# yunjinli/TRASE

Measured on AMD Instinct MI355X. Metric: views/sec (fwd+bwd), 1080p, 300k Gaussians, 32-d feat, higher is better.
Workload: dtype f32 (channel contractions: 3-product bf16-split MFMA, fp32 accumulate)

## Files before the change

include/trase_rast.h:

```cpp
#ifndef TRASE_RAST_H
#define TRASE_RAST_H

#include <stddef.h>
#include <stdint.h>

#ifdef __cplusplus
extern "C" {
#endif

typedef void* trase_stream_t;

enum {
  TRASE_OK = 0,
  TRASE_ERR_INVALID = -1,
  TRASE_ERR_UNSUPPORTED = -2,
  TRASE_ERR_WORKSPACE = -3,
  TRASE_ERR_HIP = -4
};

typedef struct TraseRastSettings {
  int32_t image_height;
  int32_t image_width;
  float tanfovx;
  float tanfovy;
  const float* bg;
  float scale_modifier;
  const float* viewmatrix;
  const float* projmatrix;
  int32_t sh_degree;
  const float* campos;
  int32_t prefiltered;
  int32_t debug;
  int32_t device;
  int32_t variant;
  int32_t tile_row_begin;
  int32_t tile_row_end;
  float feat_bg;
  int32_t reserved0;
} TraseRastSettings;

typedef enum TraseVariant {
  TRASE_VARIANT_DEPTH_GRAD = 0x100,
  TRASE_VARIANT_FEATS_BG = 0x10000,
  TRASE_VARIANT_DEPTH_NORM = 0x20000,
  TRASE_VARIANT_FEATURES_ONLY_BWD = 0x400,
  TRASE_VARIANT_VALU_BACKWARD = 0x40,
  TRASE_VARIANT_VALU_FORWARD = 0x2000,
  TRASE_VARIANT_SLOT_LISTS = 0x100000,
  TRASE_VARIANT_DEPTH32 = 0x400000,
  TRASE_VARIANT_FORWARD_ONLY = 0x800000,
  TRASE_VARIANT_SPARSE_STRIP_GRADS = 0x200000,
  TRASE_VARIANT_AB_TIMING = 0x1000,
  TRASE_VARIANT_AB_COUNT = 0x8000,
  TRASE_VARIANT_AB_ORDER_IMAGE = 0x40000,
  TRASE_VARIANT_AB_ORDER_8 = 0x80000
} TraseVariant;

typedef struct TraseRastInputs {
  int32_t P;
  int32_t M;
  int32_t F;
  const float* means3D;
  const float* shs;
  const float* sh_objs;
  const float* colors_precomp;
  const float* opacities;
  const float* scales;
  const float* rotations;
  const float* cov3D_precomp;
} TraseRastInputs;

typedef struct TraseRastOutputs {
  float* image;
  int32_t* radii;
  float* feats;
  float* depth;
} TraseRastOutputs;

typedef struct TraseRastWorkspace {
  void* geom; size_t geom_bytes;
  void* bin;  size_t bin_bytes;
  void* img;  size_t img_bytes;
  void* pre;  size_t pre_bytes;
  void* tmp;  size_t tmp_bytes;
  int64_t capacity;
} TraseRastWorkspace;

typedef struct TraseRastSizes {
  size_t geom_bytes, bin_bytes, img_bytes, pre_bytes, tmp_bytes, bwd_tmp_bytes;
} TraseRastSizes;

typedef struct TraseRastGrads {
  const float* dL_dimage;
  const float* dL_dfeats;
  const float* dL_ddepth;
  float* dL_dmeans3D;
  float* dL_dmeans2D;
  float* dL_dshs;
  float* dL_dsh_objs;
  float* dL_dcolors;
  float* dL_dopacities;
  float* dL_dscales;
  float* dL_drotations;
  float* dL_dcov3D;
} TraseRastGrads;

int trase_rast_sizes(int32_t P, int32_t W, int32_t H, int32_t F, int64_t capacity, TraseRastSizes* out);

int trase_rast_preprocess(const TraseRastSettings* s, const TraseRastInputs* in, const TraseRastOutputs* out,
                          const TraseRastWorkspace* ws, trase_stream_t stream);

int trase_rast_status(const TraseRastWorkspace* ws, int64_t status[3], trase_stream_t stream);

int trase_rast_geom_layout(int32_t P, int64_t off[6]);

int trase_rast_render(const TraseRastSettings* s, const TraseRastInputs* in, const TraseRastOutputs* out,
                      const TraseRastWorkspace* ws, trase_stream_t stream);

int trase_rast_forward(const TraseRastSettings* s, const TraseRastInputs* in, const TraseRastOutputs* out,
                       const TraseRastWorkspace* ws, trase_stream_t stream);

int trase_rast_backward(const TraseRastSettings* s, const TraseRastInputs* in, const TraseRastOutputs* out,
                        const TraseRastWorkspace* ws, const TraseRastGrads* g, trase_stream_t stream);

typedef struct TraseRastRawInputs {
  int32_t P;
  int32_t F;
  int32_t norm_features;
  const float* xyz;
  const float* d_xyz;
  const float* features_dc;
  const float* features_rest;
  const float* opacity;
  const float* scaling;
  const float* d_scaling;
  const float* rotation;
  const float* d_rotation;
  const float* gaussian_features;
  float* featn;
  const float* colors_precomp;
  const uint8_t* mask;
  const float* d_xyz_se3;
  int32_t sh_dir_undeformed;
  int32_t reserved1;
} TraseRastRawInputs;

typedef struct TraseRastRawGrads {
  const float* dL_dimage; const float* dL_dfeats; const float* dL_ddepth;
  float* dL_dxyz; float* dL_dd_xyz; float* dL_dmeans2D;
  float* dL_dfeatures_dc; float* dL_dfeatures_rest; float* dL_dopacity;
  float* dL_dscaling; float* dL_dd_scaling; float* dL_drotation; float* dL_dd_rotation;
  float* dL_dgaussian_features;
  float* dL_dcolors_precomp;
  float* dL_dd_xyz_se3;
} TraseRastRawGrads;

int trase_rast_preprocess_raw(const TraseRastSettings* s, const TraseRastRawInputs* raw, const TraseRastOutputs* out,
                              const TraseRastWorkspace* ws, trase_stream_t stream);
int trase_rast_render_raw(const TraseRastSettings* s, const TraseRastRawInputs* raw, const TraseRastOutputs* out,
                          const TraseRastWorkspace* ws, trase_stream_t stream);
int trase_rast_backward_raw(const TraseRastSettings* s, const TraseRastRawInputs* raw, const TraseRastOutputs* out,
                            const TraseRastWorkspace* ws, const TraseRastRawGrads* g, trase_stream_t stream);
int trase_rast_forward_raw(const TraseRastSettings* s, const TraseRastRawInputs* raw, const TraseRastOutputs* out,
                           const TraseRastWorkspace* ws, trase_stream_t stream);
int trase_rast_pair_sizes(int32_t P, size_t* bytes);
int trase_rast_forward_raw_pair(const TraseRastSettings* s0, const TraseRastRawInputs* raw0, const TraseRastOutputs* out0,
                                const TraseRastWorkspace* ws0, const TraseRastSettings* s1, const TraseRastRawInputs* raw1,
                                const TraseRastOutputs* out1, const TraseRastWorkspace* ws1, void* pair_ws, size_t pair_bytes,
                                trase_stream_t stream);

int trase_rast_graph_mode(int mode);
int trase_rast_graph_stats(int64_t stats[4]);

int trase_rast_backward_raw_compose(const TraseRastSettings* s, const TraseRastRawInputs* raw, const TraseRastOutputs* out,
                                    const TraseRastWorkspace* ws, const TraseRastRawGrads* g, trase_stream_t stream);
int trase_rast_zero_live_rows(const TraseRastSettings* s, const TraseRastRawInputs* raw, const TraseRastWorkspace* ws,
                              const TraseRastRawGrads* g, trase_stream_t stream);
int trase_rast_backward_raw_gaussians(const TraseRastSettings* s, const TraseRastRawInputs* raw, const TraseRastOutputs* out,
                                      const TraseRastWorkspace* ws, const TraseRastRawGrads* g, int32_t p_begin, int32_t p_end,
                                      trase_stream_t stream);

int trase_knn_sizes(int32_t N, size_t* ws_bytes);
int trase_knn_dist2(const float* points, int32_t N, float* out, void* ws, size_t ws_bytes, int32_t device,
                    trase_stream_t stream);

int trase_knn_points(const float* p1, int32_t N1, const float* p2, int32_t N2, int32_t K, int64_t* idx,
                     float* dists, void* ws, size_t ws_bytes, int32_t device, trase_stream_t stream);

typedef struct TraseMlpWeights {
  int32_t D;
  int32_t W;
  int32_t xyz_multires;
  int32_t t_multires;
  int32_t is_blender;
  int32_t is_6dof;
  int32_t variant;
  int32_t reserved;
  const float* weight[8];
  const float* bias[8];
  const float* w_warp;     const float* b_warp;
  const float* w_rotation; const float* b_rotation;
  const float* w_scaling;  const float* b_scaling;
// ... 231 lines not shown
```

trase_amd/csrc/api.hip:

```cpp
#include <stdarg.h>
#include <string.h>

#include <initializer_list>
#include <map>
#include <mutex>
#include <string>
#include <vector>

#include "common.h"

namespace trase {

static thread_local char g_err[512] = "";

void set_error(const char* fmt, ...) {
  va_list ap;
  va_start(ap, fmt);
  vsnprintf(g_err, sizeof(g_err), fmt, ap);
  va_end(ap);
}

int check_hip(hipError_t e, const char* what) {
  if (e == hipSuccess) return 0;
  set_error("HIP error %d (%s) at %s", (int)e, hipGetErrorString(e), what);
  return TRASE_ERR_HIP;
}

struct ProfRec { std::string name; hipEvent_t e0, e1; };
static std::mutex g_prof_mu;
static bool g_prof_on = false;
static int g_prof_mode = 0;
static std::vector<ProfRec*> g_prof_recs;

bool prof_on() { return g_prof_on; }

ProfScope::ProfScope(const char* n, hipStream_t s) : name(n), stream(s), rec(nullptr) {
  if (!g_prof_on) return;
  if (g_prof_mode == 2 && strncmp(n, "render_", 7) != 0) return;
  ProfRec* r = new ProfRec();
  r->name = n;
  if (hipEventCreate(&r->e0) != hipSuccess || hipEventCreate(&r->e1) != hipSuccess) { delete r; return; }
  hipEventRecord(r->e0, s);
  rec = r;
}

ProfScope::~ProfScope() {
  if (!rec) return;
  ProfRec* r = (ProfRec*)rec;
  hipEventRecord(r->e1, stream);
  std::lock_guard<std::mutex> lk(g_prof_mu);
  g_prof_recs.push_back(r);
}

static size_t geom_layout(void* ws, int P, GeomBuf& g) {
  const size_t p = (size_t)P;
  WsCursor w(ws);
  g.hdr = w.take<uint32_t>(HDR_WORDS);
  g.xy = w.take<float2>(p);
  g.conic_o = w.take<float4>(p);
  g.rgbd = w.take<float4>(p);
  g.tiles = w.take<uint32_t>(p);
  g.clamped = w.take<uint32_t>(p);
  g.geo = w.take<float4>(4 * p);
  g.ftab = w.take<uint32_t>(32 * p);
  return w.bytes();
}
static size_t bin_layout(void* ws, int64_t cap, int T, BinBuf& b) {
  WsCursor w(ws);
  b.point_list = w.take<uint32_t>((size_t)cap);
  b.pair_slot = w.take<uint32_t>((size_t)cap);
  b.ranges = w.take<uint2>((size_t)T + 1);
  return w.bytes();
}
static size_t img_layout(void* ws, int W, int H, ImgBuf& im) {
  WsCursor w(ws);
  im.final_T = w.take<float>((size_t)W * H);
  im.n_contrib = w.take<uint32_t>((size_t)W * H);
  return w.bytes();
}
static size_t pre_layout(void* ws, int P, PreBuf& t) {
  const size_t p = (size_t)(P > 0 ? P : 1), partials = p / 1024 + 2;
  WsCursor w(ws);
  sort_layout(w, t.sort, p, SORT_KEYS | SORT_VALS);
  t.offsets = w.take<uint32_t>(p);
  t.id_end = w.take<uint32_t>(p);
  t.live_ids = w.take<uint32_t>(p);
  t.block_sums = w.take<uint32_t>(3 * partials);
  t.block_R = t.block_sums + partials;
  t.block_max = t.block_R + partials;
  sort_layout(w, t.sort, p, SORT_HIST, DEPTH_MAX_DIGIT_BITS);
  return w.bytes();
}
static size_t tmp_layout(void* ws, int64_t cap, PairBuf& t) {
  const size_t n = (size_t)cap;
  WsCursor w(ws);
  sort_layout(w, t.sort, n, SORT_KEYS);
  t.sort.vals[0] = t.sort.vals[1] = nullptr;
  t.spare_vals = w.take<uint32_t>(n);
  t.pair_gauss = w.take<uint32_t>(n);
  sort_layout(w, t.sort, n, SORT_HIST);
  return w.bytes();
}
static size_t bwd_layout(void* ws, int P, int F, int64_t cap, BwdBuf& b) {
  WsCursor w(ws);
  b.acc = w.take<float>(BWD_ACC * (size_t)P);
  const size_t flags_at = w.bytes();
  b.row_flags = w.take<uint8_t>((size_t)cap);
  b.flags_bytes = w.bytes() - flags_at;
  b.rows = w.take<float>(bwd_row_stride(F) * (size_t)cap);
  return w.bytes();
}
static size_t geom_bytes(int P) { GeomBuf g; return geom_layout(nullptr, P, g); }
static size_t bin_bytes(int64_t cap, int T) { BinBuf b; return bin_layout(nullptr, cap, T, b); }
static size_t img_bytes(int W, int H) { ImgBuf im; return img_layout(nullptr, W, H, im); }
static size_t pre_bytes(int P) { PreBuf t; return pre_layout(nullptr, P, t); }
static size_t tmp_bytes(int64_t cap) { PairBuf t; return tmp_layout(nullptr, cap, t); }
static size_t bwd_tmp_bytes(int P, int F, int64_t cap) { BwdBuf b; return bwd_layout(nullptr, P, F, cap, b); }

static int list_pack_bits(const TraseRastSettings* s, int P) {
  if (s->variant & TRASE_VARIANT_SLOT_LISTS) return 0;
  int lg = 0;
  while ((1ll << lg) < (long long)P) ++lg;
  if (lg >= 28) return 0;
  return lg < 1 ? 31 : 32 - lg;
}

static int validate(const TraseRastSettings* s, const TraseRastInputs* in) {
  if (!s || !in) { set_error("null settings/inputs"); return TRASE_ERR_INVALID; }
  if (in->P < 0 || s->image_width <= 0 || s->image_height <= 0) { set_error("bad sizes"); return TRASE_ERR_INVALID; }
  if (!s->bg || !s->viewmatrix || !s->projmatrix || !s->campos) { set_error("bg/viewmatrix/projmatrix/campos are required"); return TRASE_ERR_INVALID; }
  if (in->F != 0 && in->F != 16 && in->F != 32) { set_error("feature width %d not compiled in (0,16,32)", in->F); return TRASE_ERR_UNSUPPORTED; }
  if (in->P == 0) return TRASE_OK;
  if ((in->shs == nullptr) == (in->colors_precomp == nullptr)) {
    set_error("Please provide excatly one of either SHs or precomputed colors!");
    return TRASE_ERR_INVALID;
  }
  const bool sr = in->scales != nullptr || in->rotations != nullptr;
  if ((sr && in->cov3D_precomp) || (!sr && !in->cov3D_precomp) || (sr && (!in->scales || !in->rotations))) {
    set_error("Please provide exactly one of either scale/rotation pair or precomputed 3D covariance!");
    return TRASE_ERR_INVALID;
  }
  if (!in->means3D || !in->opacities) { set_error("means3D/opacities are required"); return TRASE_ERR_INVALID; }
  if (s->sh_degree < 0 || s->sh_degree > 3) { set_error("sh_degree %d outside 0..3", s->sh_degree); return TRASE_ERR_INVALID; }
  if (in->shs && (in->M < (s->sh_degree + 1) * (s->sh_degree + 1) || in->M > 16)) {
    set_error("shs holds %d coefficients, degree %d needs %d (max 16)", in->M, s->sh_degree, (s->sh_degree + 1) * (s->sh_degree + 1));
    return TRASE_ERR_INVALID;
  }
  if (in->F > 0 && !in->sh_objs) { set_error("F>0 but sh_objs is null"); return TRASE_ERR_INVALID; }
  return TRASE_OK;
}

struct GraphEntry { std::string key; hipGraphExec_t exec; };
static std::mutex g_graph_mu;
static int g_graph_mode = [] { const char* e = getenv("TRASE_GRAPH"); return !e || !strcmp(e, "auto") ? 2 : (atoi(e) != 0 ? 1 : 0); }();
static int g_graph_auto_p = [] { const char* e = getenv("TRASE_GRAPH_AUTO_P"); return e ? atoi(e) : 200000; }();
static std::map<uint64_t, std::vector<GraphEntry>> g_graphs;
static size_t g_graph_count = 0;
static int64_t g_graph_hits = 0, g_graph_misses = 0;
static std::map<int, hipStream_t> g_capture_streams;

static uint64_t fnv1a(const std::string& s) {
  uint64_t h = 1469598103934665603ull;
  for (unsigned char c : s) { h ^= c; h *= 1099511628211ull; }
  return h;
}

static void graph_clear_locked() {
  for (auto& kv : g_graphs) for (auto& e : kv.second) hipGraphExecDestroy(e.exec);
  g_graphs.clear();
  g_graph_count = 0;
}

template <class Body>
static int run_maybe_graphed(int entry_id, std::initializer_list<std::pair<const void*, size_t>> parts, int debug, int device,
                             hipStream_t stream, int P, Body&& body) {
  if (!g_graph_mode || debug || prof_on() || (g_graph_mode == 2 && P > g_graph_auto_p)) return body(stream);
  {
    hipStreamCaptureStatus cs = hipStreamCaptureStatusNone;
    if (hipStreamIsCapturing(stream, &cs) == hipSuccess && cs != hipStreamCaptureStatusNone) return body(stream);
    (void)hipGetLastError();
  }
  std::string key((const char*)&entry_id, sizeof(entry_id));
  for (auto& p : parts) if (p.first) key.append((const char*)p.first, p.second); else key.append(p.second, '\0');
  const uint64_t h = fnv1a(key);
  std::lock_guard<std::mutex> lk(g_graph_mu);
  auto it = g_graphs.find(h);
  if (it != g_graphs.end()) {
    for (auto& e : it->second) {
      if (e.key == key) {
        ++g_graph_hits;
        return check_hip(hipGraphLaunch(e.exec, stream), "hipGraphLaunch");
      }
    }
  }
  ++g_graph_misses;
  if (g_graph_misses > 512 && g_graph_hits < g_graph_misses) { g_graph_mode = 0; graph_clear_locked(); return body(stream); }
  if (g_graph_count >= 256) graph_clear_locked();
  if (hipSetDevice(device) != hipSuccess) { (void)hipGetLastError(); return body(stream); }
  hipStream_t& cap = g_capture_streams[device];
  if (!cap && hipStreamCreateWithFlags(&cap, hipStreamNonBlocking) != hipSuccess) { cap = nullptr; (void)hipGetLastError(); return body(stream); }
  if (hipStreamBeginCapture(cap, hipStreamCaptureModeThreadLocal) != hipSuccess) { (void)hipGetLastError(); return body(stream); }
  const int rc = body(cap);
  hipGraph_t graph = nullptr;
  const hipError_t ec = hipStreamEndCapture(cap, &graph);
  if (rc != TRASE_OK || ec != hipSuccess || !graph) {
    if (graph) hipGraphDestroy(graph);
    (void)hipGetLastError();
    return body(stream);
  }
  hipGraphExec_t exec = nullptr;
  const hipError_t ei = hipGraphInstantiate(&exec, graph, nullptr, nullptr, 0);
  hipGraphDestroy(graph);
  if (ei != hipSuccess || !exec) { (void)hipGetLastError(); return body(stream); }
  g_graphs[h].push_back(GraphEntry{key, exec});
  ++g_graph_count;
  return check_hip(hipGraphLaunch(exec, stream), "hipGraphLaunch");
}

static inline bool strip_mode(const TraseRastSettings* s) { return s->tile_row_begin != 0 || s->tile_row_end != 0; }
static inline bool valu_backward(const TraseRastSettings* s) {
  return (s->variant & TRASE_VARIANT_VALU_BACKWARD) != 0 && (s->variant & TRASE_VARIANT_FEATURES_ONLY_BWD) == 0;
}

static int depth_order(const LaunchCtx& c, const TraseRastSettings* s, const GeomBuf& g, const PreBuf& t, int P, const int32_t* radii,
                       int pack_bits) {
  const DepthSortCfg cfg = depth_sort_cfg(s->variant);
  uint32_t* const flag = cfg.key_bits == 27 ? g.hdr + HDR_OVERFLOW : nullptr;
  int rc, idx = 0;
  if (strip_mode(s)) {
    rc = launch_compact_live(c, g, P, t, t.sort.keys[1 - cfg.start], t.sort.keys[cfg.start], t.sort.vals[cfg.start]);
    if (rc) return rc;
    rc = radix_sort_pairs(c, t.sort, g.hdr + (HDR_WORDS - 1), (uint32_t)P, 0, cfg.key_bits, false, &idx, cfg.digit_bits, cfg.start, DEPTH27_SAT, flag);
  } else {
    rc = radix_sort_pairs(c, t.sort, g.hdr + (HDR_WORDS - 1), (uint32_t)P, 0, cfg.key_bits, true, &idx, cfg.digit_bits, cfg.start, DEPTH27_SAT, flag);
  }
  if (rc) return rc;
  if (idx != 0) {
    set_error("internal: depth sort ended in buffer %d", idx);
    return TRASE_ERR_INVALID;
  }
  return launch_scan_tiles(c, g, t.sort.vals[0], P, t, 0xffffffffu, radii, (s->image_width + TILE - 1) / TILE,
                           (s->image_height + TILE - 1) / TILE, pack_bits);
}

enum { WS_GEOM = 1, WS_PRE = 2, WS_BIN = 4, WS_IMG = 8, WS_TMP = 16 };
static int check_ws(const TraseRastInputs* in, const TraseRastSettings* s, const TraseRastWorkspace* ws, int need) {
  if (!ws) { set_error("null workspace"); return TRASE_ERR_WORKSPACE; }
  const int gx = (s->image_width + SUB - 1) / SUB, gy = (s->image_height + SUB - 1) / SUB;
  if ((need & WS_GEOM) && (!ws->geom || ws->geom_bytes < geom_bytes(in->P))) { set_error("geom workspace missing/too small"); return TRASE_ERR_WORKSPACE; }
  if ((need & WS_PRE) && (!ws->pre || ws->pre_bytes < pre_bytes(in->P))) { set_error("pre workspace missing/too small"); return TRASE_ERR_WORKSPACE; }
  if (need & (WS_BIN | WS_TMP)) {
    if (ws->capacity < 1 || ws->capacity > 0xfffffff0ll) { set_error("capacity out of range"); return TRASE_ERR_WORKSPACE; }
  }
  if ((need & WS_BIN) && (!ws->bin || ws->bin_bytes < bin_bytes(ws->capacity, gx * gy))) { set_error("bin workspace missing/too small"); return TRASE_ERR_WORKSPACE; }
  if ((need & WS_IMG) && (!ws->img || ws->img_bytes < img_bytes(s->image_width, s->image_height))) { set_error("img workspace missing/too small"); return TRASE_ERR_WORKSPACE; }
  if ((need & WS_TMP) && (!ws->tmp || ws->tmp_bytes < tmp_bytes(ws->capacity))) { set_error("tmp workspace missing/too small"); return TRASE_ERR_WORKSPACE; }
  return TRASE_OK;
}

}

using namespace trase;

extern "C" {

const char* trase_last_error(void) { return g_err; }
const char* trase_version(void) { return "trase_amd 0.1 (gfx950)"; }

int trase_rast_sizes(int32_t P, int32_t W, int32_t H, int32_t F, int64_t capacity, TraseRastSizes* out) {
  (void)F;
  if (!out || P < 0 || W <= 0 || H <= 0 || capacity < 1) { set_error("trase_rast_sizes: bad arguments"); return TRASE_ERR_INVALID; }
  const int gx = (W + SUB - 1) / SUB, gy = (H + SUB - 1) / SUB;
  out->geom_bytes = geom_bytes(P);
  out->bin_bytes = bin_bytes(capacity, gx * gy);
  out->img_bytes = img_bytes(W, H);
  out->pre_bytes = pre_bytes(P);
  out->tmp_bytes = tmp_bytes(capacity);
  out->bwd_tmp_bytes = bwd_tmp_bytes(P, F, capacity);
  return TRASE_OK;
}

int trase_rast_geom_layout(int32_t P, int64_t off[6]) {
  if (P < 0 || !off) { set_error("trase_rast_geom_layout: bad arguments"); return TRASE_ERR_INVALID; }
  const uintptr_t base = 256;
  GeomBuf g;
  geom_layout((void*)base, P, g);
  const void* const field[6] = {g.hdr, g.xy, g.conic_o, g.rgbd, g.tiles, g.clamped};
  for (int i = 0; i < 6; ++i) off[i] = (int64_t)((uintptr_t)field[i] - base);
  return TRASE_OK;
}

int trase_rast_preprocess(const TraseRastSettings* s, const TraseRastInputs* in, const TraseRastOutputs* out,
                          const TraseRastWorkspace* ws, trase_stream_t stream_) {
  int rc = validate(s, in);
  if (rc) return rc;
  if (!out || (in->P > 0 && !out->radii)) { set_error("radii output required"); return TRASE_ERR_INVALID; }
  rc = check_ws(in, s, ws, WS_GEOM | WS_PRE);
  if (rc) return rc;
  hipStream_t stream = (hipStream_t)stream_;
  TRASE_CHECK(hipSetDevice(s->device));
  LaunchCtx c{stream, s->debug, s->variant};
  GeomBuf g; geom_layout(ws->geom, in->P, g);
  PreBuf t; pre_layout(ws->pre, in->P, t);
  if (in->P == 0) return launch_zero_bytes(g.hdr, sizeof(uint32_t) * HDR_WORDS, stream);
  const DepthSortCfg cfg = depth_sort_cfg(s->variant);
  rc = launch_preprocess_fwd(c, *s, *in, out->radii, g, t.sort.keys[strip_mode(s) ? 1 - cfg.start : cfg.start], cfg.key_bits == 27);
  if (rc) return rc;
  return depth_order(c, s, g, t, in->P, out->radii, list_pack_bits(s, in->P));
}

int trase_rast_status(const TraseRastWorkspace* ws, int64_t status[3], trase_stream_t stream_) {
  if (!ws || !ws->geom || !status) { set_error("trase_rast_status: bad arguments"); return TRASE_ERR_INVALID; }
  uint32_t h[32];
  hipStream_t stream = (hipStream_t)stream_;
  TRASE_CHECK(hipMemcpyAsync(h, ws->geom, sizeof(h), hipMemcpyDeviceToHost, stream));
  TRASE_CHECK(hipStreamSynchronize(stream));
  status[0] = h[HDR_R]; status[1] = h[HDR_OVERFLOW]; status[2] = h[HDR_R_EFF];
  if (h[16] || h[20]) {
    set_error("binning guard tripped: key flag %u (i=%u key=%u), slot flag %u (i=%u slot=%u)", h[16], h[17], h[18], h[20], h[21], h[22]);
    return TRASE_ERR_HIP;
  }
  return TRASE_OK;
}

int trase_rast_render(const TraseRastSettings* s, const TraseRastInputs* in, const TraseRastOutputs* out,
                      const TraseRastWorkspace* ws, trase_stream_t stream_) {
  int rc = validate(s, in);
  if (rc) return rc;
  if (!out || !out->image || !out->depth || (in->P > 0 && !out->radii) || (in->F > 0 && !out->feats)) { set_error("null output"); return TRASE_ERR_INVALID; }
  rc = check_ws(in, s, ws, WS_GEOM | WS_PRE | WS_BIN | WS_IMG | WS_TMP);
  if (rc) return rc;
  hipStream_t stream = (hipStream_t)stream_;
  TRASE_CHECK(hipSetDevice(s->device));
  LaunchCtx c{stream, s->debug, s->variant};
  const int gx = (s->image_width + SUB - 1) / SUB, gy = (s->image_height + SUB - 1) / SUB;
  const int T = gx * gy;
  GeomBuf g; geom_layout(ws->geom, in->P, g);
  BinBuf b; bin_layout(ws->bin, ws->capacity, T, b);
  ImgBuf im; img_layout(ws->img, s->image_width, s->image_height, im);
  PreBuf pre; pre_layout(ws->pre, in->P, pre);
  b.id_end = pre.id_end;
  PairBuf t; tmp_layout(ws->tmp, ws->capacity, t);
  const uint32_t cap = (uint32_t)ws->capacity;
  if (in->P > 0) {
    int bits = 1;
    while ((1 << bits) < T + 1) ++bits;
    const int passes = radix_passes(0, bits);
    const int final_idx = passes & 1;
    t.sort.vals[final_idx] = b.pair_slot;
    t.sort.vals[final_idx ^ 1] = t.spare_vals;
    rc = launch_emit_pairs(c, *s, g, out->radii, pre.sort.vals[0], in->P, pre, t.sort.keys[0], t.pair_gauss, cap, b.ranges,
                           t.sort.vals[0]);
    if (rc) return rc;
    int idx = 0;
    rc = radix_sort_pairs(c, t.sort, g.hdr + HDR_R_EFF, cap, 0, bits, false, &idx);
    if (rc) return rc;
    if (idx != final_idx) { set_error("internal: tile sort ended in buffer %d", idx); return TRASE_ERR_INVALID; }
    rc = launch_tile_ranges(c, t.sort.keys[idx], g.hdr + HDR_R_EFF, cap, b.ranges, T + 1, g.hdr + 16, false);
    if (rc) return rc;
    return launch_render_fwd(c, *s, *in, *out, g, b, im, t.pair_gauss, (uint32_t)cap);
  } else {
    launch_zero_bytes(b.ranges, sizeof(uint2) * ((size_t)T + 1), stream);
  }
  return launch_render_fwd(c, *s, *in, *out, g, b, im);
}

int trase_rast_forward(const TraseRastSettings* s, const TraseRastInputs* in, const TraseRastOutputs* out,
                       const TraseRastWorkspace* ws, trase_stream_t stream) {
  if (!s || !in || !out || !ws) { set_error("null argument"); return TRASE_ERR_INVALID; }
  return run_maybe_graphed(1, {{s, sizeof(*s)}, {in, sizeof(*in)}, {out, sizeof(*out)}, {ws, sizeof(*ws)}}, s->debug, s->device, (hipStream_t)stream, in->P,
                           [&](hipStream_t st) {
                             int rc = trase_rast_preprocess(s, in, out, ws, st);
                             if (rc) return rc;
                             return trase_rast_render(s, in, out, ws, st);
                           });
}

int trase_rast_graph_mode(int mode) {
  std::lock_guard<std::mutex> lk(g_graph_mu);
  g_graph_mode = mode;
  g_graph_hits = g_graph_misses = 0;
  if (!mode) graph_clear_locked();
  return TRASE_OK;
}

int trase_rast_graph_stats(int64_t stats[4]) {
  if (!stats) return TRASE_ERR_INVALID;
  std::lock_guard<std::mutex> lk(g_graph_mu);
  stats[0] = g_graph_hits; stats[1] = g_graph_misses; stats[2] = (int64_t)g_graph_count; stats[3] = g_graph_mode;
  return TRASE_OK;
}

static int backward_impl(const TraseRastSettings* s, const TraseRastInputs* in, const TraseRastOutputs* out,
                         const TraseRastWorkspace* ws, const TraseRastGrads* gr, trase_stream_t stream_);

int trase_rast_backward(const TraseRastSettings* s, const TraseRastInputs* in, const TraseRastOutputs* out,
                        const TraseRastWorkspace* ws, const TraseRastGrads* gr, trase_stream_t stream_) {
  if (!s || !in || !out || !ws || !gr) { set_error("null argument"); return TRASE_ERR_INVALID; }
  return run_maybe_graphed(2, {{s, sizeof(*s)}, {in, sizeof(*in)}, {out, sizeof(*out)}, {ws, sizeof(*ws)}, {gr, sizeof(*gr)}}, s->debug, s->device,
                           (hipStream_t)stream_, in->P, [&](hipStream_t st) { return backward_impl(s, in, out, ws, gr, st); });
}

static int backward_impl(const TraseRastSettings* s, const TraseRastInputs* in, const TraseRastOutputs* out,
                         const TraseRastWorkspace* ws, const TraseRastGrads* gr, trase_stream_t stream_) {
  int rc = validate(s, in);
  if (rc) return rc;
  if (!gr || !out || (in->P > 0 && !out->radii)) { set_error("null grads/outputs"); return TRASE_ERR_INVALID; }
  rc = check_ws(in, s, ws, WS_GEOM | WS_PRE | WS_BIN | WS_IMG);
  if (rc) return rc;
  if (!ws->tmp || ws->tmp_bytes < bwd_tmp_bytes(in->P, in->F, ws->capacity)) { set_error("backward tmp workspace too small"); return TRASE_ERR_WORKSPACE; }
  hipStream_t stream = (hipStream_t)stream_;
  TRASE_CHECK(hipSetDevice(s->device));
  LaunchCtx c{stream, s->debug, s->variant};
  const int gx = (s->image_width + SUB - 1) / SUB, gy = (s->image_height + SUB - 1) / SUB;
  GeomBuf g; geom_layout(ws->geom, in->P, g);
  BinBuf b; bin_layout(ws->bin, ws->capacity, gx * gy, b);
  ImgBuf im; img_layout(ws->img, s->image_width, s->image_height, im);
  PreBuf pre; pre_layout(ws->pre, in->P, pre);
  BwdBuf bw; bwd_layout(ws->tmp, in->P, in->F, ws->capacity, bw);
  if (in->P == 0) return TRASE_OK;
  TraseRastGrads g2 = *gr;
  if (!(s->variant & TRASE_VARIANT_DEPTH_GRAD)) g2.dL_ddepth = nullptr;
  TraseRastInputs in2 = *in;
  bool zero_feats = false;
  if (!g2.dL_dfeats) {
    in2.F = 0;
    zero_feats = g2.dL_dsh_objs != nullptr && in->F > 0;
    g2.dL_dsh_objs = nullptr;
  }
  if (zero_feats) launch_zero_bytes(gr->dL_dsh_objs, sizeof(float) * (size_t)in->F * in->P, stream);
  if ((in2.F == 32 || in2.F == 0) && !valu_backward(s)) {
    rc = launch_render_bwd_hw(c, *s, in2, g, b, im, g2, bw.rows, bw.row_flags, bw.flags_bytes, out->depth);
  } else {
    launch_zero_bytes(bw.row_flags, (size_t)ws->capacity, stream);
    rc = launch_render_bwd_gs(c, *s, in2, g, b, im, g2, bw.rows, bw.row_flags, out->depth);
  }
  if (rc) return rc;
  const int live_only = strip_mode(s) ? 1 : 0;
  if (live_only) {
    launch_zero_bytes(bw.acc, sizeof(float) * BWD_ACC * (size_t)in->P, stream);
    if (g2.dL_dsh_objs) launch_zero_bytes(g2.dL_dsh_objs, sizeof(float) * (size_t)in2.F * in->P, stream);
  }
  rc = launch_reduce_rows(c, g, pre, in->P, in2.F, bw.rows, bw.row_flags, bw.acc, g2.dL_dsh_objs, nullptr, 0, -1, -1, live_only);
  if (rc) return rc;
  return launch_preprocess_bwd(c, *s, *in, out->radii, g, bw.acc, *gr);
}

static int validate_raw(const TraseRastSettings* s, const TraseRastRawInputs* r) {
  if (!s || !r) { set_error("null settings/inputs"); return TRASE_ERR_INVALID; }
  if (r->P < 0 || s->image_width <= 0 || s->image_height <= 0) { set_error("bad sizes"); return TRASE_ERR_INVALID; }
  if (!s->bg || !s->viewmatrix || !s->projmatrix || !s->campos) { set_error("bg/viewmatrix/projmatrix/campos are required"); return TRASE_ERR_INVALID; }
  if (r->F != 0 && r->F != 16 && r->F != 32) { set_error("feature width %d not compiled in (0,16,32)", r->F); return TRASE_ERR_UNSUPPORTED; }
  if (s->sh_degree < 0 || s->sh_degree > 3) { set_error("sh_degree %d outside 0..3", s->sh_degree); return TRASE_ERR_INVALID; }
  if (r->P == 0) return TRASE_OK;
  if (!r->xyz || !r->opacity || !r->scaling || !r->rotation || (!r->colors_precomp && (!r->features_dc || !r->features_rest))) {
    set_error("raw inputs: xyz/opacity/scaling/rotation and either features_dc + features_rest or colors_precomp are required"); return TRASE_ERR_INVALID;
  }
  if (r->colors_precomp && r->sh_dir_undeformed) { set_error("raw inputs: colors_precomp and sh_dir_undeformed exclude each other"); return TRASE_ERR_INVALID; }
  if (r->d_xyz_se3 && r->d_xyz) { set_error("raw inputs: d_xyz_se3 (is_6dof) replaces d_xyz"); return TRASE_ERR_INVALID; }
  if (r->F > 0 && (!r->gaussian_features || !r->featn)) { set_error("raw inputs: gaussian_features/featn required when F > 0"); return TRASE_ERR_INVALID; }
  return TRASE_OK;
}

static TraseRastInputs raw_as_inputs(const TraseRastRawInputs* r) {
  TraseRastInputs in;
  memset(&in, 0, sizeof(in));
  in.P = r->P; in.M = 16; in.F = r->F; in.sh_objs = r->featn;
  return in;
}

int trase_rast_preprocess_raw(const TraseRastSettings* s, const TraseRastRawInputs* raw, const TraseRastOutputs* out,
                              const TraseRastWorkspace* ws, trase_stream_t stream_) {
  int rc = validate_raw(s, raw);
  if (rc) return rc;
  if (!out || (raw->P > 0 && !out->radii)) { set_error("radii output required"); return TRASE_ERR_INVALID; }
  const TraseRastInputs in = raw_as_inputs(raw);
  rc = check_ws(&in, s, ws, WS_GEOM | WS_PRE);
  if (rc) return rc;
  hipStream_t stream = (hipStream_t)stream_;
  TRASE_CHECK(hipSetDevice(s->device));
  LaunchCtx c{stream, s->debug, s->variant};
  GeomBuf g; geom_layout(ws->geom, in.P, g);
  PreBuf t; pre_layout(ws->pre, in.P, t);
  if (in.P == 0) return launch_zero_bytes(g.hdr, sizeof(uint32_t) * HDR_WORDS, stream);
  const DepthSortCfg cfg = depth_sort_cfg(s->variant);
  rc = launch_preprocess_fwd_raw(c, *s, *raw, out->radii, g, t.sort.keys[strip_mode(s) ? 1 - cfg.start : cfg.start], cfg.key_bits == 27, 0u,
                                 depth_dead_key(cfg.key_bits == 27));
  if (rc) return rc;
  return depth_order(c, s, g, t, in.P, out->radii, list_pack_bits(s, in.P));
}

struct PairSortWs { SortBufs sort; uint32_t* n_word; };
static size_t pair_ws_layout(void* ws, int P, PairSortWs& t) {
  WsCursor w(ws);
  sort_layout(w, t.sort, 2 * (size_t)(P > 0 ? P : 1));
  t.n_word = w.take<uint32_t>(4);
  return w.bytes();
}
static size_t pair_ws_bytes(int P) { PairSortWs t; return pair_ws_layout(nullptr, P, t); }
int trase_rast_pair_sizes(int32_t P, size_t* bytes) {
  if (!bytes || P < 0) { set_error("trase_rast_pair_sizes: bad arguments"); return TRASE_ERR_INVALID; }
  *bytes = pair_ws_bytes(P);
  return TRASE_OK;
}

static int forward_raw_pair_impl(const TraseRastSettings* const s[2], const TraseRastRawInputs* const raw[2], const TraseRastOutputs* const out[2],
                                 const TraseRastWorkspace* const ws[2], void* pair_ws, hipStream_t stream) {
  const int P = raw[0]->P;
  TRASE_CHECK(hipSetDevice(s[0]->device));
  const size_t n = 2 * (size_t)P;
  PairSortWs pw; pair_ws_layout(pair_ws, P, pw);
  const SortBufs& cs = pw.sort;
  uint32_t* const n_word = pw.n_word;
  launch_fill_u32(n_word, (uint32_t)n, stream);
  GeomBuf g[2];
  PreBuf t[2];
  for (int v = 0; v < 2; ++v) {
    LaunchCtx c{stream, s[v]->debug, s[v]->variant};
    geom_layout(ws[v]->geom, P, g[v]);
    pre_layout(ws[v]->pre, P, t[v]);
    const int rc = launch_preprocess_fwd_raw(c, *s[v], *raw[v], out[v]->radii, g[v], cs.keys[0] + (size_t)v * P, false,
                                             v ? 0x80000000u : 0u, v ? 0xffffffffu : 0x7fffffffu);
    if (rc) return rc;
  }
  LaunchCtx c0{stream, s[0]->debug, s[0]->variant};
  int idx = 0;
  int rc = radix_sort_pairs(c0, cs, n_word, (uint32_t)n, 0, 32, true, &idx, 8, 0);
  if (rc) return rc;
  if (idx != 0) { set_error("internal: pair depth sort ended in buffer %d", idx); return TRASE_ERR_INVALID; }
  launch_split_pair_ids(c0, cs.vals[0], P, t[0].sort.vals[0], t[1].sort.vals[0]);
  for (int v = 0; v < 2; ++v) {
    LaunchCtx c{stream, s[v]->debug, s[v]->variant};
    rc = launch_scan_tiles(c, g[v], t[v].sort.vals[0], P, t[v], 0xffffffffu, out[v]->radii, (s[v]->image_width + TILE - 1) / TILE,
                           (s[v]->image_height + TILE - 1) / TILE, list_pack_bits(s[v], P));
    if (rc) return rc;
    rc = trase_rast_render_raw(s[v], raw[v], out[v], ws[v], (trase_stream_t)stream);
    if (rc) return rc;
  }
  return TRASE_OK;
}

int trase_rast_forward_raw_pair(const TraseRastSettings* s0, const TraseRastRawInputs* raw0, const TraseRastOutputs* out0,
                                const TraseRastWorkspace* ws0, const TraseRastSettings* s1, const TraseRastRawInputs* raw1,
                                const TraseRastOutputs* out1, const TraseRastWorkspace* ws1, void* pair_ws, size_t pair_bytes,
                                trase_stream_t stream) {
  if (!s0 || !raw0 || !out0 || !ws0 || !s1 || !raw1 || !out1 || !ws1) { set_error("null argument"); return TRASE_ERR_INVALID; }
  const TraseRastSettings* s[2] = {s0, s1};
  const TraseRastRawInputs* raw[2] = {raw0, raw1};
  const TraseRastOutputs* out[2] = {out0, out1};
  const TraseRastWorkspace* ws[2] = {ws0, ws1};
  for (int v = 0; v < 2; ++v) {
    int rc = validate_raw(s[v], raw[v]);
    if (rc) return rc;
    if (raw[v]->P > 0 && !out[v]->radii) { set_error("radii output required"); return TRASE_ERR_INVALID; }
    const TraseRastInputs in = raw_as_inputs(raw[v]);
    rc = check_ws(&in, s[v], ws[v], WS_GEOM | WS_PRE);
    if (rc) return rc;
    if (strip_mode(s[v])) { set_error("trase_rast_forward_raw_pair: tile-row strips are rendered one view at a time"); return TRASE_ERR_UNSUPPORTED; }
  }
  if (raw0->P != raw1->P || s0->device != s1->device) { set_error("trase_rast_forward_raw_pair: both views render the same P Gaussians on one device"); return TRASE_ERR_INVALID; }
  if (raw0->P == 0) {
    int rc = trase_rast_forward_raw(s0, raw0, out0, ws0, stream);
    return rc ? rc : trase_rast_forward_raw(s1, raw1, out1, ws1, stream);
  }
  if (!pair_ws || pair_bytes < pair_ws_bytes(raw0->P)) { set_error("trase_rast_forward_raw_pair: pair workspace too small"); return TRASE_ERR_WORKSPACE; }
  struct { const void* p; size_t b; } extra = {pair_ws, pair_bytes};
  return run_maybe_graphed(5, {{s0, sizeof(*s0)}, {raw0, sizeof(*raw0)}, {out0, sizeof(*out0)}, {ws0, sizeof(*ws0)}, {s1, sizeof(*s1)},
                               {raw1, sizeof(*raw1)}, {out1, sizeof(*out1)}, {ws1, sizeof(*ws1)}, {&extra, sizeof(extra)}},
                           s0->debug | s1->debug, s0->device, (hipStream_t)stream, raw0->P,
                           [&](hipStream_t st) { return forward_raw_pair_impl(s, raw, out, ws, pair_ws, st); });
}

int trase_rast_render_raw(const TraseRastSettings* s, const TraseRastRawInputs* raw, const TraseRastOutputs* out,
                          const TraseRastWorkspace* ws, trase_stream_t stream) {
  int rc = validate_raw(s, raw);
  if (rc) return rc;
  TraseRastInputs in = raw_as_inputs(raw);
  static const float dummy = 0.f;
  in.means3D = &dummy; in.opacities = &dummy; in.shs = &dummy; in.scales = &dummy; in.rotations = &dummy;
  if (in.F > 0 && !in.sh_objs) { set_error("featn required"); return TRASE_ERR_INVALID; }
  return trase_rast_render(s, &in, out, ws, stream);
}

static int backward_raw_phases(const TraseRastSettings* s, const TraseRastRawInputs* raw, const TraseRastOutputs* out,
                               const TraseRastWorkspace* ws, const TraseRastRawGrads* gr, trase_stream_t stream_, int phase,
                               int p_begin, int p_end) {
  int rc = validate_raw(s, raw);
  if (rc) return rc;
  if (!gr || !out || (raw->P > 0 && !out->radii)) { set_error("null grads/outputs"); return TRASE_ERR_INVALID; }
  TraseRastInputs in = raw_as_inputs(raw);
  rc = check_ws(&in, s, ws, WS_GEOM | WS_PRE | WS_BIN | WS_IMG);
  if (rc) return rc;
  if (!ws->tmp || ws->tmp_bytes < bwd_tmp_bytes(in.P, in.F, ws->capacity)) { set_error("backward tmp workspace too small"); return TRASE_ERR_WORKSPACE; }
  if (s->variant & TRASE_VARIANT_FORWARD_ONLY) {
    set_error("backward on a forward that ran with TRASE_VARIANT_FORWARD_ONLY: its backward-only state was never stored"); return TRASE_ERR_INVALID;
  }
  const bool ranged = p_begin >= 0;
  if (ranged && (p_begin % 64 != 0 || p_end > raw->P || p_end < p_begin || (p_end != raw->P && p_end % 64 != 0))) {
    set_error("backward_raw_gaussians: [%d, %d) must start on a multiple of 64 and end on one or at P = %d", p_begin, p_end, raw->P);
    return TRASE_ERR_INVALID;
  }
  hipStream_t stream = (hipStream_t)stream_;
  TRASE_CHECK(hipSetDevice(s->device));
  LaunchCtx c{stream, s->debug, s->variant};
  const int gx = (s->image_width + SUB - 1) / SUB, gy = (s->image_height + SUB - 1) / SUB;
  GeomBuf g; geom_layout(ws->geom, in.P, g);
  BinBuf b; bin_layout(ws->bin, ws->capacity, gx * gy, b);
  ImgBuf im; img_layout(ws->img, s->image_width, s->image_height, im);
  PreBuf pre; pre_layout(ws->pre, in.P, pre);
  BwdBuf bw; bwd_layout(ws->tmp, in.P, in.F, ws->capacity, bw);
  if (in.P == 0) return TRASE_OK;
  TraseRastGrads g2;
  memset(&g2, 0, sizeof(g2));
  g2.dL_dimage = gr->dL_dimage; g2.dL_dfeats = gr->dL_dfeats;
  g2.dL_ddepth = (s->variant & TRASE_VARIANT_DEPTH_GRAD) ? gr->dL_ddepth : nullptr;
  float* d_feats = gr->dL_dgaussian_features;
  const bool no_feat_cotangent = !g2.dL_dfeats;
  if (no_feat_cotangent) {
    in.F = 0;
    d_feats = nullptr;
  }
  const bool sparse = strip_mode(s) && !ranged && (s->variant & TRASE_VARIANT_SPARSE_STRIP_GRADS) != 0;
  if (phase & 1) {
    if (no_feat_cotangent && gr->dL_dgaussian_features && raw->F > 0 && !sparse)
      launch_zero_bytes(gr->dL_dgaussian_features, sizeof(float) * (size_t)raw->F * raw->P, stream);
    if ((in.F == 32 || in.F == 0) && !valu_backward(s)) {
      rc = launch_render_bwd_hw(c, *s, in, g, b, im, g2, bw.rows, bw.row_flags, bw.flags_bytes, out->depth);
    } else {
      launch_zero_bytes(bw.row_flags, (size_t)ws->capacity, stream);
      rc = launch_render_bwd_gs(c, *s, in, g, b, im, g2, bw.rows, bw.row_flags, out->depth);
    }
    if (rc) return rc;
  }
  if (phase & 2) {
    const int live_only = (strip_mode(s) && !ranged) ? 1 : 0;
    rc = launch_reduce_rows(c, g, pre, in.P, in.F, bw.rows, bw.row_flags, bw.acc, d_feats, raw->gaussian_features, raw->norm_features,
                            ranged ? p_begin : -1, ranged ? p_end : -1, live_only);
    if (rc) return rc;
    rc = launch_preprocess_bwd_raw(c, *s, *raw, out->radii, g, bw.acc, *gr, ranged ? p_begin : 0, ranged ? p_end : raw->P,
                                   (live_only && d_feats && !sparse) ? 1 : 0, sparse ? pre.live_ids : nullptr);
// ... 118 lines not shown
```

trase_amd/csrc/binning.hip:

```cpp
#include <stdlib.h>

#include "common.h"

namespace trase {

constexpr int RS_WAVES = RS_THREADS / WAVE;
constexpr int RS_SEG = WAVE * RS_ITEMS;

__device__ __forceinline__ uint32_t dev_n(const uint32_t* n_ptr, uint32_t cap) {
  const uint32_t n = *n_ptr;
  return n < cap ? n : cap;
}

template <int DB>
__global__ __launch_bounds__(RS_THREADS) void radix_hist_kernel(const uint32_t* __restrict__ keys,
                                                                const uint32_t* __restrict__ n_ptr, uint32_t cap,
                                                                int shift, uint32_t mask, uint32_t* __restrict__ hist,
                                                                uint32_t* __restrict__ digit_total, int nb_max,
                                                                uint32_t flag_key = 0u, uint32_t* __restrict__ flag_word = nullptr,
                                                                uint32_t* __restrict__ zero_from = nullptr, uint32_t zero_words = 0u) {
  constexpr int ND = 1 << DB;
  for (uint32_t i = blockIdx.x * RS_THREADS + threadIdx.x; i < zero_words; i += gridDim.x * RS_THREADS) zero_from[i] = 0u;
  const uint32_t n = dev_n(n_ptr, cap);
  const uint32_t base = blockIdx.x * RS_TILE;
  if (base >= n) return;
  __shared__ uint32_t h[ND];
#pragma unroll
  for (int d = threadIdx.x; d < ND; d += RS_THREADS) h[d] = 0;
  __syncthreads();
  const unsigned lane = threadIdx.x & 63;
  uint32_t kk[RS_ITEMS];
#pragma unroll
  for (int i = 0; i < RS_ITEMS; ++i) {
    const uint32_t idx = base + i * RS_THREADS + threadIdx.x;
    kk[i] = idx < n ? keys[idx] : 0u;
  }
#pragma unroll
  for (int i = 0; i < RS_ITEMS; ++i) {
    const uint32_t idx = base + i * RS_THREADS + threadIdx.x;
    const bool valid = idx < n;
    if (flag_word && valid && kk[i] == flag_key) atomicOr(flag_word, 2u);
    const uint32_t dg = valid ? ((kk[i] >> shift) & mask) : 0xffffffffu;
    const uint32_t prev = (uint32_t)__shfl_up((int)dg, 1);
    const bool start = valid && (lane == 0 || prev != dg);
    const unsigned long long starts = __ballot(start);
    const unsigned long long vmask = __ballot(valid);
    if (start) {
      const unsigned long long later = (lane == 63) ? 0ull : (starts >> (lane + 1));
      const unsigned nvalid = (unsigned)__popcll(vmask);
      const unsigned next = later ? (lane + 1 + (unsigned)__builtin_ctzll(later)) : nvalid;
      atomicAdd(&h[dg], next - lane);
    }
  }
  __syncthreads();
#pragma unroll
  for (int d = threadIdx.x; d < ND; d += RS_THREADS) hist[(size_t)d * nb_max + blockIdx.x] = h[d];
}

__device__ __forceinline__ uint32_t block256_incl_scan(uint32_t v, uint32_t* part ) {
  const int lane = threadIdx.x & 63, wave = threadIdx.x >> 6;
  uint32_t x = v;
#pragma unroll
  for (int o = 1; o < 64; o <<= 1) {
    const uint32_t y = (uint32_t)__shfl_up((int)x, o);
    if (lane >= o) x += y;
  }
  if (lane == 63) part[wave] = x;
  __syncthreads();
  uint32_t add = 0;
#pragma unroll
  for (int w = 0; w < 3; ++w) add += (w < wave) ? part[w] : 0u;
  __syncthreads();
  return x + add;
}

__global__ __launch_bounds__(256) void radix_scan_kernel(const uint32_t* __restrict__ n_ptr, uint32_t cap,
                                                         uint32_t* __restrict__ hist,
                                                         uint32_t* __restrict__ digit_total, int nb_max) {
  const uint32_t n = dev_n(n_ptr, cap);
  const int nb = (int)((n + RS_TILE - 1) / RS_TILE);
  const int d = blockIdx.x;
  __shared__ uint32_t sh[256];
  __shared__ uint32_t carry;
  if (threadIdx.x == 0) carry = 0u;
  __syncthreads();
  uint32_t* row = hist + (size_t)d * nb_max;
  const int per = (nb + 255) / 256;
  const int b_lo = threadIdx.x * per, b_hi = min(b_lo + per, nb);
  uint32_t mine = 0, run;
  uint32_t incl;
  if (per <= 32) {
    uint32_t v[32];
#pragma unroll
    for (int u = 0; u < 32; ++u) v[u] = (b_lo + u < b_hi) ? row[b_lo + u] : 0u;
#pragma unroll
    for (int u = 0; u < 32; ++u) mine += v[u];
    incl = block256_incl_scan(mine, sh);
    run = incl - mine;
#pragma unroll
    for (int u = 0; u < 32; ++u) {
      if (b_lo + u < b_hi) row[b_lo + u] = run;
      run += v[u];
    }
  } else {
    for (int b = b_lo; b < b_hi; ++b) mine += row[b];
    incl = block256_incl_scan(mine, sh);
    run = incl - mine;
    for (int b = b_lo; b < b_hi; ++b) { const uint32_t v = row[b]; row[b] = run; run += v; }
  }
  if (threadIdx.x == 255) carry = incl;
  __syncthreads();
  if (threadIdx.x == 0) digit_total[d] = carry;
}

template <bool IOTA, int DB, bool SMALL = false>
__global__ __launch_bounds__(RS_THREADS) void radix_scatter_kernel(
    const uint32_t* __restrict__ keys_in, const uint32_t* __restrict__ vals_in, uint32_t* __restrict__ keys_out,
    uint32_t* __restrict__ vals_out, const uint32_t* __restrict__ n_ptr, uint32_t cap, int shift, uint32_t mask,
    const uint32_t* __restrict__ hist, const uint32_t* __restrict__ digit_total, int nb_max,
    uint32_t* __restrict__ hist_next = nullptr, int shift_next = 0, uint32_t mask_next = 0u) {
  constexpr int ND = 1 << DB;
  constexpr int DPT = ND / RS_THREADS;
  const uint32_t n = dev_n(n_ptr, cap);
  const uint32_t base = blockIdx.x * RS_TILE;
  if (base >= n) return;
  __shared__ uint32_t wcount[RS_WAVES][ND];
  const int wave = threadIdx.x >> 6;
  const unsigned lane = threadIdx.x & 63;
#pragma unroll
  for (int w = 0; w < RS_WAVES; ++w)
#pragma unroll
    for (int d = threadIdx.x; d < ND; d += RS_THREADS) wcount[w][d] = 0;
  __syncthreads();
  uint32_t k[RS_ITEMS], v[RS_ITEMS], rk[RS_ITEMS];
  const unsigned long long lt = lanemask_lt();
  volatile uint32_t* cnt = wcount[wave];
  uint32_t my_digit_total[DPT], my_hist[DPT];
  if constexpr (SMALL) {
    const int nb = (int)((n + RS_TILE - 1) / RS_TILE);
#pragma unroll
    for (int j = 0; j < DPT; ++j) {
      const uint32_t* row = hist + (size_t)(threadIdx.x * DPT + j) * nb_max;
      uint32_t before = 0, total = 0;
      for (int b0 = 0; b0 < nb; b0 += 8) {
        uint32_t v8[8];
#pragma unroll
        for (int u = 0; u < 8; ++u) v8[u] = (b0 + u < nb) ? row[b0 + u] : 0u;
#pragma unroll
        for (int u = 0; u < 8; ++u) { total += v8[u]; before += (b0 + u < (int)blockIdx.x) ? v8[u] : 0u; }
      }
      my_digit_total[j] = total; my_hist[j] = before;
    }
  } else {
#pragma unroll
  for (int j = 0; j < DPT; ++j) {
    my_digit_total[j] = digit_total[threadIdx.x * DPT + j];
    my_hist[j] = hist[(size_t)(threadIdx.x * DPT + j) * nb_max + blockIdx.x];
  }
  }
#pragma unroll
  for (int i = 0; i < RS_ITEMS; ++i) {
    const uint32_t idx = base + wave * RS_SEG + i * WAVE + lane;
    const bool valid = idx < n;
    k[i] = valid ? keys_in[idx] : 0xffffffffu;
    v[i] = valid ? (IOTA ? idx : vals_in[idx]) : 0u;
  }
#pragma unroll
  for (int i = 0; i < RS_ITEMS; ++i) {
    const uint32_t idx = base + wave * RS_SEG + i * WAVE + lane;
    const bool valid = idx < n;
    const uint32_t dg = (k[i] >> shift) & mask;
    unsigned long long peers = __ballot(valid);
    const uint32_t dg0 = __builtin_amdgcn_readfirstlane(dg);
    if (!__all(!valid || dg == dg0)) {
#pragma unroll
      for (int bit = 0; bit < DB; ++bit) {
        const bool set = (dg >> bit) & 1u;
        const unsigned long long bal = __ballot(set);
        peers &= set ? bal : ~bal;
      }
    }
    const uint32_t in_round = (uint32_t)__popcll(peers & lt);
    const uint32_t total = (uint32_t)__popcll(peers);
    uint32_t old = 0;
    if (valid) {
      old = cnt[dg];
      if (in_round == 0) cnt[dg] = old + total;
    }
    rk[i] = old + in_round;
    __builtin_amdgcn_wave_barrier();
  }
  __syncthreads();
  __shared__ uint32_t gbase[ND], lstart[ND];
  __shared__ uint32_t st_k[RS_TILE], st_v[RS_TILE];
  __shared__ uint32_t part_a[4], part_b[4];
  {
    uint32_t cnt_d[DPT], sum_l = 0, sum_g = 0;
#pragma unroll
    for (int j = 0; j < DPT; ++j) {
      const int d = threadIdx.x * DPT + j;
      uint32_t tot = 0;
#pragma unroll
      for (int w = 0; w < RS_WAVES; ++w) {
        const uint32_t c = wcount[w][d];
        wcount[w][d] = tot;
        tot += c;
      }
      cnt_d[j] = tot;
      sum_l += tot;
      sum_g += my_digit_total[j];
    }
    uint32_t run_l = block256_incl_scan(sum_l, part_a) - sum_l;
    uint32_t run_g = block256_incl_scan(sum_g, part_b) - sum_g;
#pragma unroll
    for (int j = 0; j < DPT; ++j) {
      const int d = threadIdx.x * DPT + j;
      lstart[d] = run_l;
      gbase[d] = run_g + my_hist[j];
      run_l += cnt_d[j];
      run_g += my_digit_total[j];
    }
  }
  __syncthreads();
#pragma unroll
  for (int i = 0; i < RS_ITEMS; ++i) {
    const uint32_t idx = base + wave * RS_SEG + i * WAVE + lane;
    if (idx < n) {
      const uint32_t dg = (k[i] >> shift) & mask;
      const uint32_t lp = lstart[dg] + wcount[wave][dg] + rk[i];
      st_k[lp] = k[i];
      st_v[lp] = v[i];
    }
  }
  __syncthreads();
  const uint32_t nblk = min((uint32_t)RS_TILE, n - base);
  for (uint32_t j = threadIdx.x; j < nblk; j += RS_THREADS) {
    const uint32_t kk = st_k[j];
    const uint32_t dg = (kk >> shift) & mask;
    const uint32_t dst = gbase[dg] + (j - lstart[dg]);
    keys_out[dst] = kk;
    vals_out[dst] = st_v[j];
    if constexpr (SMALL) {
      if (hist_next) {
        const uint32_t word = ((kk >> shift_next) & mask_next) * (uint32_t)nb_max + dst / RS_TILE;
        const uint32_t prev = (uint32_t)__shfl_up((int)word, 1);
        const bool start = lane == 0 || prev != word;
        const unsigned long long starts = __ballot(start), act = __ballot(true);
        if (start) {
          const unsigned long long later = (lane == 63) ? 0ull : (starts >> (lane + 1));
          const unsigned nact = (unsigned)__popcll(act);
          const unsigned next = later ? (lane + 1 + (unsigned)__builtin_ctzll(later)) : nact;
          atomicAdd(hist_next + word, next - lane);
        }
      }
    }
  }
}

__global__ __launch_bounds__(256) void zero_bytes_kernel(uint8_t* __restrict__ p, size_t bytes) {
  const size_t head = ((size_t)(-(intptr_t)p) & 15u) < bytes ? ((size_t)(-(intptr_t)p) & 15u) : bytes;
  const size_t n16 = (bytes - head) >> 4;
  uint4* q = reinterpret_cast<uint4*>(p + head);
  const size_t stride = (size_t)gridDim.x * blockDim.x, t = (size_t)blockIdx.x * blockDim.x + threadIdx.x;
  for (size_t i = t; i < n16; i += stride) q[i] = make_uint4(0u, 0u, 0u, 0u);
  const size_t tail0 = head + (n16 << 4);
  if (t < head) p[t] = 0;
  if (t < bytes - tail0) p[tail0 + t] = 0;
}
int launch_zero_bytes(void* p, size_t bytes, hipStream_t stream) {
  if (!p || bytes == 0) return TRASE_OK;
  const size_t n16 = bytes >> 4;
  const unsigned blocks = (unsigned)(n16 / 256 / 4 + 1 < 4096 ? n16 / 256 / 4 + 1 : 4096);
  hipLaunchKernelGGL(zero_bytes_kernel, dim3(blocks), dim3(256), 0, stream, (uint8_t*)p, bytes);
  return TRASE_OK;
}

__global__ void fill_u32_kernel(uint32_t* p, uint32_t v) { if (threadIdx.x == 0 && blockIdx.x == 0) *p = v; }
int launch_fill_u32(uint32_t* p, uint32_t v, hipStream_t stream) {
  hipLaunchKernelGGL(fill_u32_kernel, dim3(1), dim3(64), 0, stream, p, v);
  return TRASE_OK;
}
__global__ __launch_bounds__(256) void split_pair_ids_kernel(const uint32_t* __restrict__ sorted, int P, uint32_t* __restrict__ ids0,
                                                             uint32_t* __restrict__ ids1) {
  const int i = blockIdx.x * 256 + threadIdx.x;
  if (i >= 2 * P) return;
  const uint32_t v = sorted[i];
  if (i < P) ids0[i] = v; else ids1[i - P] = v - (uint32_t)P;
}
int launch_split_pair_ids(const LaunchCtx& c, const uint32_t* sorted, int P, uint32_t* ids0, uint32_t* ids1) {
  ProfScope ps("split_pair_ids", c.stream);
  hipLaunchKernelGGL(split_pair_ids_kernel, dim3((2 * P + 255) / 256), dim3(256), 0, c.stream, sorted, P, ids0, ids1);
  return TRASE_OK;
}

int radix_passes(int bit_lo, int bit_hi, int digit_bits) { return (bit_hi - bit_lo + digit_bits - 1) / digit_bits; }

template <int DB>
static int radix_sort_pairs_t(const LaunchCtx& c, const SortBufs& t, const uint32_t* n_ptr, uint32_t n_cap, int bit_lo, int bit_hi,
                              bool vals_are_iota, int start, int* out_idx, uint32_t flag_key, uint32_t* flag_word) {
  constexpr int ND = 1 << DB;
  int cur = start;
  const int nb = (int)((n_cap + RS_TILE - 1) / RS_TILE);
  if (nb > t.nb_max) { set_error("radix_sort_pairs: nb %d > nb_max %d", nb, t.nb_max); return TRASE_ERR_WORKSPACE; }
  const int passes = radix_passes(bit_lo, bit_hi, DB);
  if (passes > RS_MAX_PASSES) return TRASE_ERR_INVALID;
  static const bool small_off = [] { const char* e = getenv("TRASE_SORT_SMALL"); return e && atoi(e) == 0; }();
  if (nb <= RS_SMALL_NB && t.hist_copies >= passes && !small_off) {
    const size_t hw = (size_t)ND * t.nb_max;
    for (int p = 0; p < passes; ++p) {
      const int shift = bit_lo + DB * p;
      const int nbits = (bit_hi - shift) < DB ? (bit_hi - shift) : DB;
      const uint32_t mask = (1u << nbits) - 1u;
      const int shift_n = shift + DB;
      const int nbits_n = (bit_hi - shift_n) < DB ? (bit_hi - shift_n) : DB;
      uint32_t* hist_p = t.hist + hw * p;
      uint32_t* hist_n = (p + 1 < passes) ? t.hist + hw * (p + 1) : nullptr;
      if (p == 0) {
        ProfScope ps("radix_hist", c.stream);
        hipLaunchKernelGGL(radix_hist_kernel<DB>, dim3(nb), dim3(RS_THREADS), 0, c.stream, t.keys[cur], n_ptr, n_cap, shift, mask, hist_p,
                           t.digit_total, t.nb_max, flag_key, flag_word, t.hist + hw, (uint32_t)(hw * (passes - 1)));
      }
      TRASE_POST_LAUNCH("radix_hist", c.stream, c.debug);
      {
        ProfScope ps("radix_scatter", c.stream);
        const uint32_t mask_n = hist_n ? ((1u << nbits_n) - 1u) : 0u;
        if (vals_are_iota && p == 0)
          hipLaunchKernelGGL((radix_scatter_kernel<true, DB, true>), dim3(nb), dim3(RS_THREADS), 0, c.stream, t.keys[cur], t.vals[cur],
                             t.keys[cur ^ 1], t.vals[cur ^ 1], n_ptr, n_cap, shift, mask, hist_p, t.digit_total, t.nb_max, hist_n, shift_n, mask_n);
        else
          hipLaunchKernelGGL((radix_scatter_kernel<false, DB, true>), dim3(nb), dim3(RS_THREADS), 0, c.stream, t.keys[cur], t.vals[cur],
                             t.keys[cur ^ 1], t.vals[cur ^ 1], n_ptr, n_cap, shift, mask, hist_p, t.digit_total, t.nb_max, hist_n, shift_n, mask_n);
      }
      TRASE_POST_LAUNCH("radix_scatter", c.stream, c.debug);
      cur ^= 1;
    }
    *out_idx = cur;
    return TRASE_OK;
  }
  for (int p = 0; p < passes; ++p) {
    const int shift = bit_lo + DB * p;
    const int nbits = (bit_hi - shift) < DB ? (bit_hi - shift) : DB;
    const uint32_t mask = (1u << nbits) - 1u;
    uint32_t* dt = t.digit_total + ND * p;
    uint32_t* vout = t.vals[cur ^ 1];
    {
      ProfScope ps("radix_hist", c.stream);
      hipLaunchKernelGGL(radix_hist_kernel<DB>, dim3(nb), dim3(RS_THREADS), 0, c.stream, t.keys[cur], n_ptr, n_cap, shift,
                         mask, t.hist, dt, t.nb_max, flag_key, p == 0 ? flag_word : (uint32_t*)nullptr);
    }
    TRASE_POST_LAUNCH("radix_hist", c.stream, c.debug);
    {
      ProfScope ps("radix_scan", c.stream);
      hipLaunchKernelGGL(radix_scan_kernel, dim3(ND), dim3(256), 0, c.stream, n_ptr, n_cap, t.hist, dt, t.nb_max);
    }
    TRASE_POST_LAUNCH("radix_scan", c.stream, c.debug);
    {
      ProfScope ps("radix_scatter", c.stream);
      if (vals_are_iota && p == 0)
        hipLaunchKernelGGL((radix_scatter_kernel<true, DB>), dim3(nb), dim3(RS_THREADS), 0, c.stream, t.keys[cur],
                           t.vals[cur], t.keys[cur ^ 1], vout, n_ptr, n_cap, shift, mask, t.hist, dt, t.nb_max);
      else
        hipLaunchKernelGGL((radix_scatter_kernel<false, DB>), dim3(nb), dim3(RS_THREADS), 0, c.stream, t.keys[cur],
                           t.vals[cur], t.keys[cur ^ 1], vout, n_ptr, n_cap, shift, mask, t.hist, dt, t.nb_max);
    }
    TRASE_POST_LAUNCH("radix_scatter", c.stream, c.debug);
    cur ^= 1;
  }
  *out_idx = cur;
  return TRASE_OK;
}

int radix_sort_pairs(const LaunchCtx& c, const SortBufs& t, const uint32_t* n_ptr, uint32_t n_cap, int bit_lo, int bit_hi,
                     bool vals_are_iota, int* out_idx, int digit_bits, int start, uint32_t flag_key, uint32_t* flag_word) {
  if (digit_bits == 9) return radix_sort_pairs_t<9>(c, t, n_ptr, n_cap, bit_lo, bit_hi, vals_are_iota, start, out_idx, flag_key, flag_word);
  if (digit_bits == 8) return radix_sort_pairs_t<8>(c, t, n_ptr, n_cap, bit_lo, bit_hi, vals_are_iota, start, out_idx, flag_key, flag_word);
  set_error("radix_sort_pairs: digit_bits %d", digit_bits);
  return TRASE_ERR_INVALID;
}

constexpr int SC_THREADS = 256;
constexpr int SC_ITEMS = 4;
constexpr int SC_TILE = SC_THREADS * SC_ITEMS;

__global__ __launch_bounds__(SC_THREADS) void compact_count_kernel(const uint32_t* __restrict__ tiles, int P,
                                                                   uint32_t* __restrict__ block_cnt) {
  const int base = blockIdx.x * SC_TILE + threadIdx.x * SC_ITEMS;
  uint32_t c = 0;
  if (base + SC_ITEMS <= P) {
    const uint4 t = *reinterpret_cast<const uint4*>(tiles + base);
    c = (t.x != 0) + (t.y != 0) + (t.z != 0) + (t.w != 0);
  } else {
#pragma unroll
    for (int k = 0; k < SC_ITEMS; ++k) c += (base + k < P && tiles[base + k] != 0) ? 1u : 0u;
  }
#pragma unroll
  for (int o = 32; o > 0; o >>= 1) c += (uint32_t)__shfl_xor((int)c, o);
  __shared__ uint32_t part[SC_THREADS / 64];
  if ((threadIdx.x & 63) == 0) part[threadIdx.x >> 6] = c;
  __syncthreads();
  if (threadIdx.x == 0) block_cnt[blockIdx.x] = part[0] + part[1] + part[2] + part[3];
}

__global__ __launch_bounds__(SC_THREADS) void compact_scatter_kernel(const uint32_t* __restrict__ tiles,
                                                                     const uint32_t* __restrict__ keys_raw, int P,
                                                                     const uint32_t* __restrict__ block_cnt, int nblocks,
                                                                     uint32_t* __restrict__ keys_out,
                                                                     uint32_t* __restrict__ ids_out,
                                                                     uint32_t* __restrict__ live_ids,
                                                                     uint32_t* __restrict__ hdr) {
  __shared__ uint32_t sh[SC_THREADS / 64];
  __shared__ uint32_t sh2[SC_THREADS / 64];
  uint32_t before = 0, total = 0;
  for (int b = threadIdx.x; b < nblocks; b += SC_THREADS) {
    const uint32_t v = block_cnt[b];
    total += v;
    before += (b < (int)blockIdx.x) ? v : 0u;
  }
#pragma unroll
  for (int o = 32; o > 0; o >>= 1) { before += (uint32_t)__shfl_xor((int)before, o); total += (uint32_t)__shfl_xor((int)total, o); }
  if ((threadIdx.x & 63) == 0) { sh[threadIdx.x >> 6] = before; sh2[threadIdx.x >> 6] = total; }
  __syncthreads();
  before = sh[0] + sh[1] + sh[2] + sh[3];
  total = sh2[0] + sh2[1] + sh2[2] + sh2[3];
  __syncthreads();
  if (blockIdx.x == 0 && threadIdx.x == 0) hdr[HDR_WORDS - 1] = total;
  const int base = blockIdx.x * SC_TILE + threadIdx.x * SC_ITEMS;
  uint32_t t[SC_ITEMS], k[SC_ITEMS];
  uint32_t mine = 0;
#pragma unroll
  for (int j = 0; j < SC_ITEMS; ++j) {
    const bool in = base + j < P;
    t[j] = in ? tiles[base + j] : 0u;
    k[j] = in ? keys_raw[base + j] : 0u;
    mine += t[j] != 0;
  }
  __shared__ uint32_t part[4];
  const uint32_t incl = block256_incl_scan(mine, part);
  uint32_t live_before = before + incl - mine;
#pragma unroll
  for (int j = 0; j < SC_ITEMS; ++j) {
    const int i = base + j;
    if (i >= P) break;
    if (t[j] != 0) {
      keys_out[live_before] = k[j];
      ids_out[live_before] = (uint32_t)i;
      live_ids[live_before] = (uint32_t)i;
      ++live_before;
    } else {
      ids_out[total + (uint32_t)i - live_before] = (uint32_t)i;
    }
  }
}

int launch_compact_live(const LaunchCtx& c, const GeomBuf& g, int P, const PreBuf& t, const uint32_t* keys_raw,
                        uint32_t* keys_out, uint32_t* ids_out) {
  const int nblocks = (P + SC_TILE - 1) / SC_TILE;
  {
    ProfScope ps("compact_live", c.stream);
    hipLaunchKernelGGL(compact_count_kernel, dim3(nblocks), dim3(SC_THREADS), 0, c.stream, g.tiles, P, t.block_sums);
    hipLaunchKernelGGL(compact_scatter_kernel, dim3(nblocks), dim3(SC_THREADS), 0, c.stream, g.tiles, keys_raw, P, t.block_sums,
                       nblocks, keys_out, ids_out, t.live_ids, g.hdr);
  }
  TRASE_POST_LAUNCH("compact_live", c.stream, c.debug);
  return TRASE_OK;
}

__device__ __forceinline__ uint32_t block_incl_scan(uint32_t v, uint32_t* sh ) {
  sh[threadIdx.x] = v;
  __syncthreads();
  for (int s = 1; s < SC_THREADS; s <<= 1) {
    const uint32_t add = (threadIdx.x >= (unsigned)s) ? sh[threadIdx.x - s] : 0u;
    __syncthreads();
    sh[threadIdx.x] += add;
    __syncthreads();
  }
  return sh[threadIdx.x];
}

__global__ __launch_bounds__(SC_THREADS) void scan_partial_kernel(const uint32_t* __restrict__ tiles,
                                                                  const uint32_t* __restrict__ ids, int P,
                                                                  uint32_t* __restrict__ offsets,
                                                                  uint32_t* __restrict__ block_sums,
                                                                  const int32_t* __restrict__ radii,
                                                                  const float2* __restrict__ xy, int gx, int gy,
                                                                  uint32_t* __restrict__ block_R,
                                                                  uint32_t* __restrict__ block_max,
                                                                  const uint32_t* __restrict__ n_live_ptr) {
  __shared__ uint32_t sh[SC_THREADS];
  const int base = blockIdx.x * SC_TILE + threadIdx.x * SC_ITEMS;
  const int n_live = min(P, (int)*n_live_ptr);
  uint32_t area = 0;
  int rad_[SC_ITEMS];
  float2 c_[SC_ITEMS];
  uint32_t id_[SC_ITEMS];
#pragma unroll
  for (int i = 0; i < SC_ITEMS; ++i) {
    const int n = blockIdx.x * SC_TILE + i * SC_THREADS + threadIdx.x;
    rad_[i] = (n < P) ? radii[n] : 0;
    c_[i] = (n < P) ? xy[n] : make_float2(0.f, 0.f);
    id_[i] = (base + i < n_live) ? ids[base + i] : 0u;
  }
#pragma unroll
  for (int i = 0; i < SC_ITEMS; ++i) {
    int x0, y0, x1, y1;
    tile_rect(c_[i].x, c_[i].y, rad_[i] > 0 ? rad_[i] : 1, gx, gy, x0, y0, x1, y1);
    area += rad_[i] > 0 ? (uint32_t)((x1 - x0) * (y1 - y0)) : 0u;
  }
  const uint32_t area_incl = block_incl_scan(area, sh);
  if (threadIdx.x == SC_THREADS - 1) block_R[blockIdx.x] = area_incl;
  __syncthreads();
  uint32_t v[SC_ITEMS];
  uint32_t sum = 0, mx = 0;
#pragma unroll
  for (int i = 0; i < SC_ITEMS; ++i) {
    const int r = base + i;
    v[i] = (r < n_live) ? tiles[id_[i]] : 0u;
    mx = max(mx, v[i]);
    sum += v[i];
    v[i] = sum;
  }
  {
#pragma unroll
    for (int o = 32; o > 0; o >>= 1) mx = max(mx, (uint32_t)__shfl_xor((int)mx, o));
    __shared__ uint32_t shm[SC_THREADS / 64];
    if ((threadIdx.x & 63) == 0) shm[threadIdx.x >> 6] = mx;
    __syncthreads();
    if (threadIdx.x == 0) {
      uint32_t m = shm[0];
      for (int w = 1; w < SC_THREADS / 64; ++w) m = max(m, shm[w]);
      block_max[blockIdx.x] = m;
// ... 390 lines not shown
```

trase_amd/csrc/common.h:

```cpp
#pragma once

#include <hip/hip_runtime.h>
#include <stdint.h>
#include <stdio.h>

#include "../../include/trase_rast.h"
#include "gs_math.h"

namespace trase {

constexpr int WAVE = 64;

template <int CTRL, int ROW_MASK = 0xf>
__device__ __forceinline__ float dpp_f(float v) {
  return __builtin_bit_cast(float, __builtin_amdgcn_update_dpp(0, __builtin_bit_cast(int, v), CTRL, ROW_MASK, 0xf, false));
}

__device__ __forceinline__ float wave_sum_lane63(float v) {
  v += dpp_f<0x111>(v);
  v += dpp_f<0x112>(v);
  v += dpp_f<0x114>(v);
  v += dpp_f<0x118>(v);
  v += dpp_f<0x142, 0xa>(v);
  v += dpp_f<0x143, 0xc>(v);
// ... 56 lines not shown
               TRASE_SCAN2_STEP("v_mul_f32_dpp", "row_shr:2 row_mask:0xf bank_mask:0xf")
               TRASE_SCAN2_STEP("v_mul_f32_dpp", "row_shr:4 row_mask:0xf bank_mask:0xf")
               TRASE_SCAN2_STEP("v_mul_f32_dpp", "row_shr:8 row_mask:0xf bank_mask:0xf")
               TRASE_SCAN2_STEP("v_mul_f32_dpp", "row_bcast:15 row_mask:0xa bank_mask:0xf")
               "v_mul_f32_dpp %0, %0, %0 row_bcast:31 row_mask:0xc bank_mask:0xf\n\t"
               "v_mul_f32_dpp %1, %1, %1 row_bcast:31 row_mask:0xc bank_mask:0xf"
               : "+v"(a), "+v"(b));
}
__device__ __forceinline__ void wave_scan_add2_out_asm(float a, float b, float& oa, float& ob) {
  asm volatile("s_nop 1\n\t"
               "v_add_f32_dpp %0, %2, %2 row_shr:1 row_mask:0xf bank_mask:0xf bound_ctrl:0\n\t"
               "v_add_f32_dpp %1, %3, %3 row_shr:1 row_mask:0xf bank_mask:0xf bound_ctrl:0\n\ts_nop 0\n\t"
               TRASE_SCAN2_STEP("v_add_f32_dpp", "row_shr:2 row_mask:0xf bank_mask:0xf")
               TRASE_SCAN2_STEP("v_add_f32_dpp", "row_shr:4 row_mask:0xf bank_mask:0xf")
               TRASE_SCAN2_STEP("v_add_f32_dpp", "row_shr:8 row_mask:0xf bank_mask:0xf")
               TRASE_SCAN2_STEP("v_add_f32_dpp", "row_bcast:15 row_mask:0xa bank_mask:0xf")
               "v_add_f32_dpp %0, %0, %0 row_bcast:31 row_mask:0xc bank_mask:0xf\n\t"
               "v_add_f32_dpp %1, %1, %1 row_bcast:31 row_mask:0xc bank_mask:0xf"
               : "=&v"(oa), "=&v"(ob) : "v"(a), "v"(b));
}
__device__ __forceinline__ void wave_scan_add2_asm(float& a, float& b) {
  asm volatile("s_nop 1\n\t"
               TRASE_SCAN2_STEP("v_add_f32_dpp", "row_shr:1 row_mask:0xf bank_mask:0xf")
               TRASE_SCAN2_STEP("v_add_f32_dpp", "row_shr:2 row_mask:0xf bank_mask:0xf")
               TRASE_SCAN2_STEP("v_add_f32_dpp", "row_shr:4 row_mask:0xf bank_mask:0xf")
               TRASE_SCAN2_STEP("v_add_f32_dpp", "row_shr:8 row_mask:0xf bank_mask:0xf")
               TRASE_SCAN2_STEP("v_add_f32_dpp", "row_bcast:15 row_mask:0xa bank_mask:0xf")
               "v_add_f32_dpp %0, %0, %0 row_bcast:31 row_mask:0xc bank_mask:0xf\n\t"
               "v_add_f32_dpp %1, %1, %1 row_bcast:31 row_mask:0xc bank_mask:0xf"
               : "+v"(a), "+v"(b));
}
#undef TRASE_SCAN2_STEP

constexpr float LOG2_ALPHA_MIN = -7.994353436858858f;
struct PairPoly { float k0, kj, ki, kjj, kii, kij, thr; };

__device__ __forceinline__ PairPoly pair_poly(float2 gxy, float4 co, float bx, float by) {
  constexpr float L = 1.4426950408889634f;
  const float rx = gxy.x - bx, ry = gxy.y - by;
  const float A = co.x, B = co.y, C = co.z;
  PairPoly k;
  const float lo = __log2f(co.w);
  k.k0 = fmaf(L, fmaf(-0.5f, fmaf(A * rx, rx, C * ry * ry), -(B * rx) * ry), lo);
  k.kj = L * fmaf(A, rx, B * ry);
  k.ki = L * fmaf(C, ry, B * rx);
  k.kjj = -0.5f * L * A;
  k.kii = -0.5f * L * C;
  k.kij = -L * B;
  const float M = fabsf(k.k0) + 7.0f * (fabsf(k.kj) + fabsf(k.ki)) + 49.0f * (fabsf(k.kjj) + fabsf(k.kii) + fabsf(k.kij));
  k.thr = fmaf(9.5e-7f, M, lo);
  return k;
}
__device__ __forceinline__ float poly_row_base(const PairPoly& k, float i, float ii) { return fmaf(ii, k.kii, fmaf(i, k.ki, k.k0)); }
__device__ __forceinline__ float poly_row_slope(const PairPoly& k, float i) { return fmaf(i, k.kij, k.kj); }
__device__ __forceinline__ float poly_eval(const PairPoly& k, float base, float slope, float j) {
  return fmaf(j, fmaf(j, k.kjj, slope), base);
}

__device__ __forceinline__ int xcd_block(int b, int nb) {
#ifdef TRASE_NO_XCD_MAP
  return b;
#else
  const int x = b & 7, loc = b >> 3, q = nb >> 3, r = nb & 7;
  return x * q + (x < r ? x : r) + loc;
#endif
}

template <int B>
__device__ __forceinline__ void blocked_tile(int i, int gx, int gy, int& tx, int& ty) {
  const int band = i / (B * gx), rem = i - band * (B * gx);
  const int hb = min(B, gy - band * B);
  const int ncol = (gx + B - 1) / B;
  const int sc = min(rem / (hb * B), ncol - 1);
  const int r2 = rem - sc * hb * B;
  const int wb = min(B, gx - sc * B);
  ty = band * B + r2 / wb;
  tx = sc * B + r2 - (r2 / wb) * wb;
}

__device__ __forceinline__ float wave_shr1(float v, float ident) { return dpp_fill<0x138>(v, ident); }

__device__ __forceinline__ float readlane_f(float v, int lane) {
  return __builtin_bit_cast(float, __builtin_amdgcn_readlane(__builtin_bit_cast(int, v), lane));
}

__device__ __forceinline__ float wave_sum_all(float v) { return readlane_f(wave_sum_lane63(v), 63); }

__device__ __forceinline__ unsigned lane_id() { return __builtin_amdgcn_mbcnt_hi(~0u, __builtin_amdgcn_mbcnt_lo(~0u, 0u)); }

__device__ __forceinline__ unsigned long long lanemask_lt() {
  const unsigned l = lane_id();
  return (l == 0) ? 0ull : (~0ull >> (64 - l));
}

__device__ __forceinline__ void atomic_add_f32(float* p, float v) { unsafeAtomicAdd(p, v); }

void set_error(const char* fmt, ...);
int check_hip(hipError_t e, const char* what);

struct ProfScope {
  ProfScope(const char* name, hipStream_t stream);
  ~ProfScope();
  const char* name; hipStream_t stream; void* rec;
};
bool prof_on();

#define TRASE_CHECK(expr)                                  \
  do {                                                     \
    int _rc = ::trase::check_hip((expr), #expr);           \
    if (_rc != 0) return _rc;                              \
  } while (0)

#define TRASE_POST_LAUNCH(name, stream, debug)                                          \
  do {                                                                                  \
    int _rc = ::trase::check_hip(hipGetLastError(), name);                              \
    if (_rc != 0) return _rc;                                                           \
    if (debug) {                                                                        \
      if ((debug) > 1) fprintf(stderr, "[trase] %s\n", name);                           \
      _rc = ::trase::check_hip(hipStreamSynchronize(stream), name " (debug sync)");     \
      if (_rc != 0) return _rc;                                                         \
    }                                                                                   \
  } while (0)

static inline size_t align_up(size_t x, size_t a = 256) { return (x + a - 1) / a * a; }

static inline void strip_subtile_rows(const TraseRastSettings& s, int& lo, int& hi) {
  const int gy8 = (s.image_height + SUB - 1) / SUB;
  lo = 0; hi = gy8;
  if (s.tile_row_begin != 0 || s.tile_row_end != 0) {
    lo = 2 * s.tile_row_begin; hi = 2 * s.tile_row_end;
    if (lo < 0) lo = 0;
    if (hi > gy8) hi = gy8;
    if (hi < lo) hi = lo;
  }
}

struct WsCursor {
  explicit WsCursor(void* ws) : base((uintptr_t)ws) {}
  template <class T> T* take(size_t n) {
    const size_t o = off;
    off += align_up(sizeof(T) * n);
    return base ? (T*)(base + o) : nullptr;
  }
  size_t bytes() const { return off; }
  uintptr_t base;
  size_t off = 0;
};
template <class T> size_t array_layout(void* ws, size_t n, T*& p) {
  WsCursor w(ws);
  p = w.take<T>(n);
  return w.bytes();
}

enum { HDR_R = 0, HDR_OVERFLOW = 1, HDR_R_EFF = 2, HDR_PACK = 3, HDR_WORDS = 64 };
__device__ __forceinline__ uint32_t list_id(uint32_t v, uint32_t jb) { return v >> jb; }
__device__ __forceinline__ uint32_t list_slot(uint32_t v, uint32_t jb, const uint32_t* id_end, const uint32_t* tiles) {
  const uint32_t id = v >> jb;
  return id_end[id] - tiles[id] + (v & ((1u << jb) - 1u));
}

struct GeomBuf {
  uint32_t* hdr;
  float2* xy;
  float4* conic_o;
  float4* rgbd;
  uint32_t* tiles;
  uint32_t* clamped;
  float4* geo;
  uint32_t* ftab;
};
struct BinBuf {
  uint32_t* point_list;
  uint32_t* pair_slot;
  uint2* ranges;
  const uint32_t* id_end = nullptr;
};
struct ImgBuf {
  float* final_T;
  uint32_t* n_contrib;
};
struct SortBufs {
  uint32_t* keys[2];
  uint32_t* vals[2];
  uint32_t* hist;
  uint32_t* digit_total;
  int nb_max;
  int hist_copies;
};
#ifndef TRASE_RS_ITEMS
#define TRASE_RS_ITEMS 8
#endif
constexpr int RS_THREADS = 256, RS_ITEMS = TRASE_RS_ITEMS;
constexpr int RS_TILE = RS_THREADS * RS_ITEMS;
constexpr int RS_MAX_PASSES = 8;
inline int rs_blocks(size_t n) { return (int)((n + RS_TILE - 1) / RS_TILE); }
constexpr int RS_SMALL_NB = 16;
constexpr int RS_SMALL_COPIES = 4;
inline int rs_hist_copies(int nb) { return nb <= RS_SMALL_NB ? RS_SMALL_COPIES : 1; }
enum { SORT_KEYS = 1, SORT_VALS = 2, SORT_HIST = 4, SORT_ALL = 7 };
inline void sort_layout(WsCursor& w, SortBufs& s, size_t n, int parts = SORT_ALL, int digit_bits = 8, int hist_copies = 0) {
  if (parts & SORT_KEYS) for (int i = 0; i < 2; ++i) s.keys[i] = w.take<uint32_t>(n);
  if (parts & SORT_VALS) for (int i = 0; i < 2; ++i) s.vals[i] = w.take<uint32_t>(n);
  if (!(parts & SORT_HIST)) return;
  const size_t digits = (size_t)1 << digit_bits;
  s.nb_max = rs_blocks(n);
  s.hist_copies = hist_copies ? hist_copies : rs_hist_copies(s.nb_max);
  s.hist = w.take<uint32_t>(digits * s.nb_max * s.hist_copies);
  s.digit_total = w.take<uint32_t>(digits * RS_MAX_PASSES);
}
struct PreBuf {
  SortBufs sort;
  uint32_t* offsets;
  uint32_t* id_end;
  uint32_t* block_sums;
  uint32_t* block_R;
  uint32_t* block_max;
  uint32_t* live_ids;
};
struct PairBuf {
  SortBufs sort;
  uint32_t* spare_vals;
  uint32_t* pair_gauss;
};
constexpr int BWD_ACC = 12;
enum { ACC_NDCX = 0, ACC_NDCY = 1, ACC_CA = 2, ACC_CB = 3, ACC_CC = 4, ACC_OP = 5, ACC_R = 6, ACC_G = 7, ACC_B = 8, ACC_D = 9 };

struct BwdBuf {
  float* acc;
  uint8_t* row_flags;
  float* rows;
  size_t flags_bytes;
};
static inline int bwd_row_floats(int F) { return F + 12; }
#ifndef TRASE_ROW_STRIDE32
#define TRASE_ROW_STRIDE32 44
#endif
constexpr int bwd_row_stride(int F) { return F == 32 ? TRASE_ROW_STRIDE32 : F + 12; }

struct LaunchCtx { hipStream_t stream; int debug; int variant; };

typedef float f4v __attribute__((ext_vector_type(4)));
__device__ __forceinline__ float4 ld_stream(const float4* p) {
  const f4v q = __builtin_nontemporal_load(reinterpret_cast<const f4v*>(p));
  return make_float4(q.x, q.y, q.z, q.w);
}
__device__ __forceinline__ void st_stream(float4* p, const float4& v) {
  const f4v q = {v.x, v.y, v.z, v.w};
  __builtin_nontemporal_store(q, reinterpret_cast<f4v*>(p));
}

__device__ __forceinline__ void split_pk(float a, float b, unsigned& hi, unsigned& lo) {
  asm("v_cvt_pk_bf16_f32 %0, %1, %2" : "=v"(hi) : "v"(a), "v"(b));
  const float ra = a - __uint_as_float(hi << 16), rb = b - __uint_as_float(hi & 0xffff0000u);
  asm("v_cvt_pk_bf16_f32 %0, %1, %2" : "=v"(lo) : "v"(ra), "v"(rb));
}
__device__ __forceinline__ float4 split_rgbd(float r, float g, float b, float d) {
  unsigned h01, l01, h23, l23;
  split_pk(r, g, h01, l01);
  split_pk(b, d, h23, l23);
  return make_float4(__uint_as_float(h01), __uint_as_float(h23), __uint_as_float(l01), __uint_as_float(l23));
}
int launch_feature_table(const LaunchCtx& c, const float* feats, const uint32_t* tiles, int P, uint32_t* ftab);

int launch_preprocess_fwd(const LaunchCtx& c, const TraseRastSettings& s, const TraseRastInputs& in, int32_t* radii,
                          const GeomBuf& g, uint32_t* depth_keys, bool key27);
int launch_preprocess_bwd(const LaunchCtx& c, const TraseRastSettings& s, const TraseRastInputs& in, const int32_t* radii,
                          const GeomBuf& g, const float* acc, const TraseRastGrads& gr);


int launch_preprocess_bwd_raw(const LaunchCtx& c, const TraseRastSettings& s, const TraseRastRawInputs& raw,
                              const int32_t* radii, const GeomBuf& g, const float* acc, const TraseRastRawGrads& gr,
                              int p_begin = 0, int p_end = -1, int zero_dead_feats = 0, const uint32_t* live_ids = nullptr);
int launch_zero_live_rows(const LaunchCtx& c, const GeomBuf& g, const PreBuf& pre, int P, int F, const TraseRastRawGrads& gr);

int radix_sort_pairs(const LaunchCtx& c, const SortBufs& t, const uint32_t* n_ptr, uint32_t n_cap, int bit_lo, int bit_hi,
                     bool vals_are_iota, int* out_idx, int digit_bits = 8, int start = 0, uint32_t flag_key = 0u,
                     uint32_t* flag_word = nullptr);
int launch_zero_bytes(void* p, size_t bytes, hipStream_t stream);
int launch_fill_u32(uint32_t* p, uint32_t v, hipStream_t stream);
constexpr int LABEL_SUMS_MAX = 128;
struct LabelSumsWs { float* slabs; float* total; int32_t* slot; };
size_t label_sums_layout(void* ws, int N, int D, int S, LabelSumsWs& w);
int launch_label_sums(const float* X, int N, int D, const int32_t* ids, const int32_t* sel, int S, const LabelSumsWs& w, hipStream_t stream);
int launch_evaluate(const TraseEvalFrame& f, const float* final_T, hipStream_t stream);
int launch_split_pair_ids(const LaunchCtx& c, const uint32_t* sorted, int P, uint32_t* ids0, uint32_t* ids1);
int radix_passes(int bit_lo, int bit_hi, int digit_bits = 8);
struct DepthSortCfg { int key_bits, digit_bits, passes, start; };
inline DepthSortCfg depth_sort_cfg(int variant) {
  return (variant & TRASE_VARIANT_DEPTH32) ? DepthSortCfg{32, 8, 4, 0} : DepthSortCfg{27, 9, 3, 1};
}
constexpr int DEPTH_MAX_DIGIT_BITS = 9;
constexpr uint32_t DEPTH27_BASE = 0x3e4ccccdu, DEPTH27_SAT = 0x07fffffeu, DEPTH27_DEAD = 0x07ffffffu;
__host__ __device__ inline uint32_t depth_sort_key(float z, bool key27) {
  const uint32_t bits = __builtin_bit_cast(uint32_t, z);
  if (!key27) return bits;
  const uint32_t b = bits - DEPTH27_BASE;
  return b < DEPTH27_SAT ? b : DEPTH27_SAT;
}
inline uint32_t depth_dead_key(bool key27) { return key27 ? DEPTH27_DEAD : 0xffffffffu; }
int launch_preprocess_fwd_raw(const LaunchCtx& c, const TraseRastSettings& s, const TraseRastRawInputs& raw, int32_t* radii,
                              const GeomBuf& g, uint32_t* depth_keys, bool key27, uint32_t key_or = 0u, uint32_t key_dead = 0xffffffffu);

int launch_compact_live(const LaunchCtx& c, const GeomBuf& g, int P, const PreBuf& t, const uint32_t* keys_raw,
                        uint32_t* keys_out, uint32_t* ids_out);
int launch_scan_tiles(const LaunchCtx& c, const GeomBuf& g, const uint32_t* sorted_ids, int P, const PreBuf& t, uint32_t cap,
                      const int32_t* radii, int gx, int gy, int pack_bits = 0);
int launch_emit_pairs(const LaunchCtx& c, const TraseRastSettings& s, const GeomBuf& g, const int32_t* radii,
                      const uint32_t* sorted_ids, int P, const PreBuf& t, uint32_t* keys, uint32_t* pair_gauss, uint32_t cap,
                      uint2* ranges_to_clear = nullptr, uint32_t* vals = nullptr);
int launch_reduce_rows(const LaunchCtx& c, const GeomBuf& g, const PreBuf& pre, int P, int F, const float* rows,
                       const uint8_t* row_flags, float* acc, float* d_feats, const float* raw_feats = nullptr,
                       int norm_features = 0, int id_begin = -1, int id_end = -1, int live_only = 0);
int launch_tile_ranges(const LaunchCtx& c, const uint32_t* keys, const uint32_t* n_ptr, uint32_t cap, uint2* ranges, int T,
                       uint32_t* dbg = nullptr, bool clear = true);

int launch_render_fwd(const LaunchCtx& c, const TraseRastSettings& s, const TraseRastInputs& in, const TraseRastOutputs& out,
                      const GeomBuf& g, const BinBuf& b, const ImgBuf& im, const uint32_t* pair_gauss = nullptr,
                      uint32_t cap = 0);
int launch_render_fwd_mf(const LaunchCtx& c, const TraseRastSettings& s, const TraseRastInputs& in, const TraseRastOutputs& out,
                         const GeomBuf& g, const BinBuf& b, const ImgBuf& im, const uint32_t* pair_gauss, uint32_t cap);
int launch_render_bwd_gs(const LaunchCtx& c, const TraseRastSettings& s, const TraseRastInputs& in, const GeomBuf& g,
                         const BinBuf& b, const ImgBuf& im, const TraseRastGrads& gr, float* rows, uint8_t* row_flags,
                         const float* out_depth = nullptr);
int launch_render_bwd_hw(const LaunchCtx& c, const TraseRastSettings& s, const TraseRastInputs& in, const GeomBuf& g,
                         const BinBuf& b, const ImgBuf& im, const TraseRastGrads& gr, float* rows, uint8_t* row_flags,
                         size_t flag_bytes, const float* out_depth = nullptr);

}
```

trase_amd/csrc/preprocess.hip:

```cpp
#include "common.h"

namespace trase {

__device__ __forceinline__ void load_view(const float* __restrict__ vm, const float* __restrict__ pm,
                                          const float* __restrict__ cam, View& v) {
#pragma unroll
  for (int i = 0; i < 16; ++i) { v.V[i] = vm[i]; v.PM[i] = pm[i]; }
  v.cam[0] = cam[0]; v.cam[1] = cam[1]; v.cam[2] = cam[2];
}

struct PreArgs {
  const float* means3D; const float* shs; const float* colors; const float* opac; const float* scales;
  const float* rots; const float* cov3d; const float* vm; const float* pm; const float* cam;
  int P, M, deg, W, H;
  float tanx, tany, mod;
  int sy_lo, sy_hi;
  int key27;
};

__device__ __forceinline__ void fill_view(const PreArgs& a, View& v) {
  load_view(a.vm, a.pm, a.cam, v);
  v.tanx = a.tanx; v.tany = a.tany;
  v.fx = (float)a.W / (2.0f * a.tanx); v.fy = (float)a.H / (2.0f * a.tany);
  v.mod = a.mod; v.W = a.W; v.H = a.H;
  v.gx = (a.W + TILE - 1) / TILE; v.gy = (a.H + TILE - 1) / TILE;
  v.deg = a.deg;
}

template <bool USE_COV, bool USE_SH>
__global__ __launch_bounds__(256) void preprocess_fwd_kernel(PreArgs a, int32_t* __restrict__ radii,
                                                             float2* __restrict__ xy, float4* __restrict__ conic_o,
                                                             float4* __restrict__ rgbd, float4* __restrict__ geo, uint32_t* __restrict__ tiles,
                                                             uint32_t* __restrict__ clamped,
                                                             uint32_t* __restrict__ depth_keys,
                                                             uint32_t* __restrict__ hdr) {
  const int gi = blockIdx.x * blockDim.x + threadIdx.x;
  if (gi == 0) {
#pragma unroll
    for (int k = 0; k < HDR_WORDS - 1; ++k) hdr[k] = 0u;
    hdr[HDR_WORDS - 1] = (uint32_t)a.P;
  }
  const bool active = gi < a.P;
  const int i = active ? gi : a.P - 1;
  View v;
  fill_view(a, v);
  const float p[3] = {a.means3D[3 * i], a.means3D[3 * i + 1], a.means3D[3 * i + 2]};
  float sc[3] = {0.f, 0.f, 0.f}, q[4] = {0.f, 0.f, 0.f, 0.f}, cv[6] = {0.f, 0.f, 0.f, 0.f, 0.f, 0.f};
  if (USE_COV) {
#pragma unroll
    for (int k = 0; k < 6; ++k) cv[k] = a.cov3d[6 * i + k];
  } else {
    sc[0] = a.scales[3 * i]; sc[1] = a.scales[3 * i + 1]; sc[2] = a.scales[3 * i + 2];
    const float4 qq = reinterpret_cast<const float4*>(a.rots)[i];
    q[0] = qq.x; q[1] = qq.y; q[2] = qq.z; q[3] = qq.w;
  }
  float shl[48];
  float col[3] = {0.f, 0.f, 0.f};
  if (USE_SH) {
    const int n3 = 3 * ncoef(a.deg);
    const float* src = a.shs + (size_t)i * a.M * 3;
    if (a.M == 16) {
      const float4* s4 = reinterpret_cast<const float4*>(src);
#pragma unroll
      for (int k = 0; k < 12; ++k) {
        const float4 t = s4[k];
        shl[4 * k] = t.x; shl[4 * k + 1] = t.y; shl[4 * k + 2] = t.z; shl[4 * k + 3] = t.w;
      }
#pragma unroll
      for (int k = 0; k < 48; ++k) shl[k] = (k < n3) ? shl[k] : 0.f;
    } else {
#pragma unroll
      for (int k = 0; k < 48; ++k) shl[k] = (k < n3) ? src[k] : 0.f;
    }
  } else {
#pragma unroll
    for (int k = 0; k < 48; ++k) shl[k] = 0.f;
    col[0] = a.colors[3 * i]; col[1] = a.colors[3 * i + 1]; col[2] = a.colors[3 * i + 2];
  }
  Splat o;
  const bool vis = splat_forward<USE_COV, USE_SH>(v, p, sc, q, cv, shl, col, o) && active;
  if (active) radii[i] = vis ? o.radius : 0;
  uint32_t live = 0;
  const float opac = a.opac[i];
  if (vis) {
    const SubtileCull cull = subtile_cull_setup(o.px, o.py, o.ca, o.cb, o.cc, opac);
    for (int sy = max(2 * o.y0, a.sy_lo); sy < min(2 * o.y1, a.sy_hi) && sy * SUB < a.H; ++sy) {
      int c0, c1;
      subtile_row_live(cull, sy, a.W, a.H, 2 * o.x0, 2 * o.x1, c0, c1);
      live += (uint32_t)(c1 - c0);
    }
  }
  if (active) {
    tiles[i] = live;
    depth_keys[i] = (vis && live) ? depth_sort_key(o.depth, a.key27 != 0) : (a.key27 ? DEPTH27_DEAD : 0xffffffffu);
  }
  if (vis) {
    xy[i] = make_float2(o.px, o.py);
    conic_o[i] = make_float4(o.ca, o.cb, o.cc, opac);
    rgbd[i] = make_float4(o.rgb[0], o.rgb[1], o.rgb[2], o.depth);
    geo[4 * (size_t)i + 0] = make_float4(o.px, o.py, 0.f, __int_as_float(o.radius));
    geo[4 * (size_t)i + 1] = make_float4(o.ca, o.cb, o.cc, opac);
    geo[4 * (size_t)i + 2] = make_float4(o.rgb[0], o.rgb[1], o.rgb[2], o.depth);
    geo[4 * (size_t)i + 3] = split_rgbd(o.rgb[0], o.rgb[1], o.rgb[2], o.depth);
    clamped[i] = o.clamped;
  }
}

static void fill_pre_args(PreArgs& a, const TraseRastSettings& s, const TraseRastInputs& in) {
  a.means3D = in.means3D; a.shs = in.shs; a.colors = in.colors_precomp; a.opac = in.opacities;
  a.scales = in.scales; a.rots = in.rotations; a.cov3d = in.cov3D_precomp;
  a.vm = s.viewmatrix; a.pm = s.projmatrix; a.cam = s.campos;
  a.P = in.P; a.M = in.M; a.deg = s.sh_degree; a.W = s.image_width; a.H = s.image_height;
  a.tanx = s.tanfovx; a.tany = s.tanfovy; a.mod = s.scale_modifier;
  strip_subtile_rows(s, a.sy_lo, a.sy_hi);
}

int launch_preprocess_fwd(const LaunchCtx& c, const TraseRastSettings& s, const TraseRastInputs& in, int32_t* radii,
                          const GeomBuf& g, uint32_t* depth_keys, bool key27) {
  PreArgs a;
  fill_pre_args(a, s, in);
  a.key27 = key27 ? 1 : 0;
  const dim3 grid((in.P + 255) / 256), block(256);
  const bool cov = in.cov3D_precomp != nullptr, sh = in.shs != nullptr;
  {
    ProfScope ps("preprocess_fwd", c.stream);
#define TRASE_PRE_FWD(C, S) hipLaunchKernelGGL((preprocess_fwd_kernel<C, S>), grid, block, 0, c.stream, a, radii, g.xy, g.conic_o, g.rgbd, g.geo, g.tiles, g.clamped, depth_keys, g.hdr)
    if (cov) { if (sh) TRASE_PRE_FWD(true, true); else TRASE_PRE_FWD(true, false); }
    else { if (sh) TRASE_PRE_FWD(false, true); else TRASE_PRE_FWD(false, false); }
#undef TRASE_PRE_FWD
  }
  TRASE_POST_LAUNCH("preprocess_fwd", c.stream, c.debug);
  if (in.F == 32) return launch_feature_table(c, in.sh_objs, g.tiles, in.P, g.ftab);
  return TRASE_OK;
}

__global__ __launch_bounds__(256) void feature_table_kernel(const float* __restrict__ feats, const uint32_t* __restrict__ tiles,
                                                            int P, uint32_t* __restrict__ ftab) {
  const int idx = blockIdx.x * blockDim.x + threadIdx.x;
  if (idx >= P * 8) return;
  const int g = idx >> 3, l = idx & 7;
  if (tiles[g] == 0) return;
  const float4 v = reinterpret_cast<const float4*>(feats + (size_t)g * 32)[l];
  unsigned h01, l01, h23, l23;
  split_pk(v.x, v.y, h01, l01);
  split_pk(v.z, v.w, h23, l23);
  *reinterpret_cast<uint2*>(ftab + (size_t)g * 32 + 2 * l) = make_uint2(h01, h23);
  *reinterpret_cast<uint2*>(ftab + (size_t)g * 32 + 16 + 2 * l) = make_uint2(l01, l23);
}
int launch_feature_table(const LaunchCtx& c, const float* feats, const uint32_t* tiles, int P, uint32_t* ftab) {
  if (P <= 0) return TRASE_OK;
  {
    ProfScope ps("feature_table", c.stream);
    hipLaunchKernelGGL(feature_table_kernel, dim3((P * 8 + 255) / 256), dim3(256), 0, c.stream, feats, tiles, P, ftab);
  }
  TRASE_POST_LAUNCH("feature_table", c.stream, c.debug);
  return TRASE_OK;
}

struct PreBwdOut {
  float* d_means3D; float* d_means2D; float* d_shs; float* d_colors; float* d_opac; float* d_scales;
  float* d_rots; float* d_cov3d;
};

template <bool USE_COV, bool USE_SH>
__global__ __launch_bounds__(256) void preprocess_bwd_kernel(PreArgs a, const int32_t* __restrict__ radii,
                                                             const uint32_t* __restrict__ clamped,
                                                             const uint32_t* __restrict__ tiles,
                                                             const float* __restrict__ acc, PreBwdOut o) {
  const int i = blockIdx.x * blockDim.x + threadIdx.x;
  if (i >= a.P) return;
  const bool vis = radii[i] > 0 && tiles[i] > 0;
  SplatGradOut go;
  float dsh[48];
#pragma unroll
  for (int k = 0; k < 48; ++k) dsh[k] = 0.f;
  SplatGradIn gi;
  gi.d_ndcx = gi.d_ndcy = gi.d_ca = gi.d_cb = gi.d_cc = gi.d_depth = 0.f;
  gi.d_rgb[0] = gi.d_rgb[1] = gi.d_rgb[2] = 0.f;
  float d_op = 0.f;
#pragma unroll
  for (int k = 0; k < 3; ++k) { go.d_p[k] = 0.f; go.d_scale[k] = 0.f; }
#pragma unroll
  for (int k = 0; k < 4; ++k) go.d_quat[k] = 0.f;
#pragma unroll
  for (int k = 0; k < 6; ++k) go.d_cov[k] = 0.f;
  if (vis) {
    const float4* r4 = reinterpret_cast<const float4*>(acc + (size_t)i * BWD_ACC);
    const float4 r0 = r4[0], r1 = r4[1], r2 = r4[2];
    gi.d_ndcx = r0.x; gi.d_ndcy = r0.y; gi.d_ca = r0.z; gi.d_cb = r0.w;
    gi.d_cc = r1.x; d_op = r1.y; gi.d_rgb[0] = r1.z; gi.d_rgb[1] = r1.w;
    gi.d_rgb[2] = r2.x; gi.d_depth = r2.y;
    View v;
    fill_view(a, v);
    const float p[3] = {a.means3D[3 * i], a.means3D[3 * i + 1], a.means3D[3 * i + 2]};
    float sc[3] = {0.f, 0.f, 0.f}, q[4] = {0.f, 0.f, 0.f, 0.f}, cv[6] = {0.f, 0.f, 0.f, 0.f, 0.f, 0.f};
    if (USE_COV) {
#pragma unroll
      for (int k = 0; k < 6; ++k) cv[k] = a.cov3d[6 * i + k];
    } else {
      sc[0] = a.scales[3 * i]; sc[1] = a.scales[3 * i + 1]; sc[2] = a.scales[3 * i + 2];
      const float4 qq = reinterpret_cast<const float4*>(a.rots)[i];
      q[0] = qq.x; q[1] = qq.y; q[2] = qq.z; q[3] = qq.w;
    }
    float shl[48];
    if (USE_SH) {
      const int n3 = 3 * ncoef(a.deg);
      const float* src = a.shs + (size_t)i * a.M * 3;
      if (a.M == 16) {
        const float4* s4 = reinterpret_cast<const float4*>(src);
#pragma unroll
        for (int k = 0; k < 12; ++k) {
          const float4 t = s4[k];
          shl[4 * k] = t.x; shl[4 * k + 1] = t.y; shl[4 * k + 2] = t.z; shl[4 * k + 3] = t.w;
        }
#pragma unroll
        for (int k = 0; k < 48; ++k) shl[k] = (k < n3) ? shl[k] : 0.f;
      } else {
#pragma unroll
        for (int k = 0; k < 48; ++k) shl[k] = (k < n3) ? src[k] : 0.f;
      }
    } else {
#pragma unroll
      for (int k = 0; k < 48; ++k) shl[k] = 0.f;
    }
    splat_backward<USE_COV, USE_SH>(v, p, sc, q, cv, shl, USE_SH ? clamped[i] : 0u, gi, go, dsh);
  }
  if (o.d_means3D) { o.d_means3D[3 * i] = go.d_p[0]; o.d_means3D[3 * i + 1] = go.d_p[1]; o.d_means3D[3 * i + 2] = go.d_p[2]; }
  if (o.d_means2D) { o.d_means2D[3 * i] = gi.d_ndcx; o.d_means2D[3 * i + 1] = gi.d_ndcy; o.d_means2D[3 * i + 2] = 0.f; }
  if (o.d_opac) o.d_opac[i] = d_op;
  if (!USE_COV) {
    if (o.d_scales) { o.d_scales[3 * i] = go.d_scale[0]; o.d_scales[3 * i + 1] = go.d_scale[1]; o.d_scales[3 * i + 2] = go.d_scale[2]; }
    if (o.d_rots) reinterpret_cast<float4*>(o.d_rots)[i] = make_float4(go.d_quat[0], go.d_quat[1], go.d_quat[2], go.d_quat[3]);
  } else if (o.d_cov3d) {
#pragma unroll
    for (int k = 0; k < 6; ++k) o.d_cov3d[6 * i + k] = go.d_cov[k];
  }
  if (!USE_SH) {
    if (o.d_colors) { o.d_colors[3 * i] = gi.d_rgb[0]; o.d_colors[3 * i + 1] = gi.d_rgb[1]; o.d_colors[3 * i + 2] = gi.d_rgb[2]; }
  } else if (o.d_shs) {
    float* dst = o.d_shs + (size_t)i * a.M * 3;
    if (a.M == 16) {
      float4* d4 = reinterpret_cast<float4*>(dst);
#pragma unroll
      for (int k = 0; k < 12; ++k) d4[k] = make_float4(dsh[4 * k], dsh[4 * k + 1], dsh[4 * k + 2], dsh[4 * k + 3]);
    } else {
      const int m3 = a.M * 3;
#pragma unroll
      for (int k = 0; k < 48; ++k)
        if (k < m3) dst[k] = dsh[k];
    }
  }
}

int launch_preprocess_bwd(const LaunchCtx& c, const TraseRastSettings& s, const TraseRastInputs& in, const int32_t* radii,
                          const GeomBuf& g, const float* acc, const TraseRastGrads& gr) {
  PreArgs a;
  fill_pre_args(a, s, in);
  PreBwdOut o;
  o.d_means3D = gr.dL_dmeans3D; o.d_means2D = gr.dL_dmeans2D; o.d_shs = in.shs ? gr.dL_dshs : nullptr;
  o.d_colors = in.colors_precomp ? gr.dL_dcolors : nullptr; o.d_opac = gr.dL_dopacities;
  o.d_scales = in.cov3D_precomp ? nullptr : gr.dL_dscales; o.d_rots = in.cov3D_precomp ? nullptr : gr.dL_drotations;
  o.d_cov3d = in.cov3D_precomp ? gr.dL_dcov3D : nullptr;
  const dim3 grid((in.P + 255) / 256), block(256);
  const bool cov = in.cov3D_precomp != nullptr, sh = in.shs != nullptr;
  {
    ProfScope ps("preprocess_bwd", c.stream);
#define TRASE_PRE_BWD(C, S) hipLaunchKernelGGL((preprocess_bwd_kernel<C, S>), grid, block, 0, c.stream, a, radii, g.clamped, g.tiles, acc, o)
    if (cov) { if (sh) TRASE_PRE_BWD(true, true); else TRASE_PRE_BWD(true, false); }
    else { if (sh) TRASE_PRE_BWD(false, true); else TRASE_PRE_BWD(false, false); }
#undef TRASE_PRE_BWD
  }
  TRASE_POST_LAUNCH("preprocess_bwd", c.stream, c.debug);
  return TRASE_OK;
}
// ... 3 lines not shown
```

trase_amd/csrc/preprocess_raw.hip:

```cpp
#include "common.h"

namespace trase {

struct RawFwdArgs {
  const float* xyz; const float* d_xyz; const float* f_dc; const float* f_rest; const float* opacity;
  const float* scaling; const float* d_scaling; const float* rotation; const float* d_rotation;
  const float* features; float* featn;
  int write_featn;
  const float* vm; const float* pm; const float* cam;
  int P, F, deg, W, H, norm_features;
  float tanx, tany, mod;
  int sy_lo, sy_hi;
  int strip;
  int p_begin, p_end;
  int key27;
  uint32_t key_or, key_dead;
  const float* colors;
  const uint8_t* mask;
  const float* se3;
  int sh_dir_raw;
  int fwd_only;
};

__device__ __forceinline__ void raw_view(const RawFwdArgs& a, View& v) {
#pragma unroll
  for (int i = 0; i < 16; ++i) { v.V[i] = a.vm[i]; v.PM[i] = a.pm[i]; }
  v.cam[0] = a.cam[0]; v.cam[1] = a.cam[1]; v.cam[2] = a.cam[2];
  v.tanx = a.tanx; v.tany = a.tany;
  v.fx = (float)a.W / (2.0f * a.tanx); v.fy = (float)a.H / (2.0f * a.tany);
  v.mod = a.mod; v.W = a.W; v.H = a.H;
  v.gx = (a.W + TILE - 1) / TILE; v.gy = (a.H + TILE - 1) / TILE;
  v.deg = a.deg;
}

struct Activated { float p[3], sc[3], q[4], opac, qn[4], inv_n, es[3], sig; };

template <bool INFER = false>
__device__ __forceinline__ void activate(const RawFwdArgs& a, int i, Activated& o) {
#pragma unroll
  for (int k = 0; k < 3; ++k) {
    o.p[k] = a.xyz[3 * i + k] + (a.d_xyz ? a.d_xyz[3 * i + k] : 0.f);
    o.es[k] = __expf(a.scaling[3 * i + k]);
    o.sc[k] = o.es[k] + (a.d_scaling ? a.d_scaling[3 * i + k] : 0.f);
  }
  if constexpr (INFER) {
    if (a.se3) {
      const float4* M = reinterpret_cast<const float4*>(a.se3) + 4 * (size_t)i;
      const float x = a.xyz[3 * i], y = a.xyz[3 * i + 1], z = a.xyz[3 * i + 2];
      const float4 r0 = M[0], r1 = M[1], r2 = M[2], r3 = M[3];
      const float h0 = r0.x * x + r0.y * y + r0.z * z + r0.w, h1 = r1.x * x + r1.y * y + r1.z * z + r1.w;
      const float h2 = r2.x * x + r2.y * y + r2.z * z + r2.w, h3 = r3.x * x + r3.y * y + r3.z * z + r3.w;
      o.p[0] = h0 / h3; o.p[1] = h1 / h3; o.p[2] = h2 / h3;
    }
  }
  const float4 r = reinterpret_cast<const float4*>(a.rotation)[i];
  const float n = sqrtf(r.x * r.x + r.y * r.y + r.z * r.z + r.w * r.w);
  o.inv_n = 1.0f / fmaxf(n, 1e-12f);
  o.qn[0] = r.x * o.inv_n; o.qn[1] = r.y * o.inv_n; o.qn[2] = r.z * o.inv_n; o.qn[3] = r.w * o.inv_n;
  float4 dq = make_float4(0.f, 0.f, 0.f, 0.f);
  if (a.d_rotation) dq = reinterpret_cast<const float4*>(a.d_rotation)[i];
  o.q[0] = o.qn[0] + dq.x; o.q[1] = o.qn[1] + dq.y; o.q[2] = o.qn[2] + dq.z; o.q[3] = o.qn[3] + dq.w;
  o.sig = 1.0f / (1.0f + __expf(-a.opacity[i]));
  o.opac = o.sig;
}

constexpr int REST_W = 45;
constexpr int REST_SLAB = 64 * REST_W;
constexpr int REST_Q = REST_SLAB / 4 / 64 + 1;

__device__ __forceinline__ void wave_lds_sync() {
  __builtin_amdgcn_fence(__ATOMIC_RELEASE, "wavefront");
  __builtin_amdgcn_wave_barrier();
  __builtin_amdgcn_fence(__ATOMIC_ACQUIRE, "wavefront");
}

struct RestRegs { float4 q[REST_Q]; };

__device__ __forceinline__ void rest_rows_load(const float* __restrict__ base, int row0, int P, bool aligned16, RestRegs& r) {
  const int lane = threadIdx.x & 63;
  const int nfl = min(64, P - row0) * REST_W;
  const float* src = base + (size_t)row0 * REST_W;
#pragma unroll
  for (int k = 0; k < REST_Q; ++k) {
    const int e = 4 * (k * 64 + lane);
    float4 v = make_float4(0.f, 0.f, 0.f, 0.f);
    if (aligned16 && e + 3 < nfl) v = *reinterpret_cast<const float4*>(src + e);
    else {
      if (e < nfl) v.x = src[e];
      if (e + 1 < nfl) v.y = src[e + 1];
      if (e + 2 < nfl) v.z = src[e + 2];
      if (e + 3 < nfl) v.w = src[e + 3];
    }
    r.q[k] = v;
  }
}

__device__ __forceinline__ void rest_rows_to_lds(const RestRegs& r, float* slab) {
  const int lane = threadIdx.x & 63;
#pragma unroll
  for (int k = 0; k < REST_Q; ++k) {
    const int e = 4 * (k * 64 + lane);
    if (e < REST_SLAB) *reinterpret_cast<float4*>(slab + e) = r.q[k];
  }
  wave_lds_sync();
}

__device__ __forceinline__ void load_sh_split(const RawFwdArgs& a, int i, const float* slab, float shl[48]) {
  const int n3 = 3 * ncoef(a.deg);
  const float* dc = a.f_dc + 3 * (size_t)i;
  shl[0] = dc[0]; shl[1] = dc[1]; shl[2] = dc[2];
  const float* row = slab + (threadIdx.x & 63) * REST_W;
#pragma unroll
  for (int k = 3; k < 48; ++k) shl[k] = (k < n3) ? row[k - 3] : 0.f;
}

__device__ __forceinline__ void rest_rows_store(float* __restrict__ base, int row0, int P, bool aligned16, const float* slab) {
  const int lane = threadIdx.x & 63;
  const int nfl = min(64, P - row0) * REST_W;
  float* dst = base + (size_t)row0 * REST_W;
#pragma unroll
  for (int k = 0; k < REST_Q; ++k) {
    const int e = 4 * (k * 64 + lane);
    if (e >= REST_SLAB) continue;
    const float4 v = *reinterpret_cast<const float4*>(slab + e);
    if (aligned16 && e + 3 < nfl) *reinterpret_cast<float4*>(dst + e) = v;
    else {
      if (e < nfl) dst[e] = v.x;
      if (e + 1 < nfl) dst[e + 1] = v.y;
      if (e + 2 < nfl) dst[e + 2] = v.z;
      if (e + 3 < nfl) dst[e + 3] = v.w;
    }
  }
}

#ifndef TRASE_RAW_BLOCK
#define TRASE_RAW_BLOCK 64
#endif
constexpr int RAW_BLOCK = TRASE_RAW_BLOCK;

template <int F, int BLOCK, bool INFER = false>
__global__ __launch_bounds__(BLOCK) void preprocess_fwd_raw_kernel(RawFwdArgs a, int32_t* __restrict__ radii,
                                                                 float2* __restrict__ xy, float4* __restrict__ conic_o,
                                                                 float4* __restrict__ rgbd, float4* __restrict__ geo, uint32_t* __restrict__ ftab,
                                                                 uint32_t* __restrict__ tiles,
                                                                 uint32_t* __restrict__ clamped,
                                                                 uint32_t* __restrict__ depth_keys,
                                                                 uint32_t* __restrict__ hdr) {
#ifdef TRASE_RAW_SETPRIO
  __builtin_amdgcn_s_setprio(3);
#endif
  const int gi = blockIdx.x * blockDim.x + threadIdx.x;
  if (gi == 0) {
#pragma unroll
    for (int k = 0; k < HDR_WORDS - 1; ++k) hdr[k] = 0u;
    hdr[HDR_WORDS - 1] = (uint32_t)a.P;
  }
  const bool active = gi < a.P;
  const int i = active ? gi : a.P - 1;
  constexpr bool strip = BLOCK != RAW_BLOCK;
#ifdef TRASE_RAW_NO_SLAB
  constexpr bool noslab = true;
#else
  constexpr bool noslab = strip;
#endif
  __shared__ __attribute__((aligned(16))) float slabs[noslab ? 1 : BLOCK / 64][noslab ? 4 : REST_SLAB];
  float* const slab = slabs[noslab ? 0 : (threadIdx.x >> 6)];
  const int row0 = gi & ~63;
  if (row0 >= a.P) return;
  const bool rest16 = ((reinterpret_cast<uintptr_t>(a.f_rest) & 15) == 0);
  const bool precol = INFER && a.colors != nullptr;
  RestRegs rr;
  if (!noslab && !precol) rest_rows_load(a.f_rest, row0, a.P, rest16, rr);
  View v;
  raw_view(a, v);
  Activated act;
  activate<INFER>(a, i, act);
  const bool masked_out = INFER && a.mask != nullptr && a.mask[i] == 0;
  float shl[48];
  const float cv[6] = {0.f, 0.f, 0.f, 0.f, 0.f, 0.f}, col[3] = {0.f, 0.f, 0.f};
  Splat o;
  bool vis = splat_forward<false, false>(v, act.p, act.sc, act.q, cv, shl, col, o) && active && !masked_out;
  if (active) radii[i] = vis ? o.radius : 0;
  uint32_t live = 0;
  if (vis) {
    const SubtileCull cull = subtile_cull_setup(o.px, o.py, o.ca, o.cb, o.cc, act.opac);
    for (int sy = max(2 * o.y0, a.sy_lo); sy < min(2 * o.y1, a.sy_hi) && sy * SUB < a.H; ++sy) {
      int c0, c1;
      subtile_row_live(cull, sy, a.W, a.H, 2 * o.x0, 2 * o.x1, c0, c1);
      live += (uint32_t)(c1 - c0);
    }
  }
  if (active) {
    tiles[i] = live;
    depth_keys[i] = (vis && live) ? (depth_sort_key(o.depth, a.key27 != 0) | a.key_or) : a.key_dead;
  }
  const bool want = vis && (live != 0 || !strip);
  if (!noslab && !precol) {
    rest_rows_to_lds(rr, slab);
  }
  if (strip) {
    if (vis && !live) xy[i] = make_float2(o.px, o.py);
  }
  if (want && precol) {
    o.rgb[0] = a.colors[3 * (size_t)i]; o.rgb[1] = a.colors[3 * (size_t)i + 1]; o.rgb[2] = a.colors[3 * (size_t)i + 2];
    o.clamped = 0u;
  } else if (want) {
    if (!noslab) {
      load_sh_split(a, i, slab, shl);
    } else {
      const int n3 = 3 * ncoef(a.deg);
      const float* dc = a.f_dc + 3 * (size_t)i;
      const float* rw = a.f_rest + (size_t)i * REST_W;
      shl[0] = dc[0]; shl[1] = dc[1]; shl[2] = dc[2];
#pragma unroll
      for (int k = 3; k < 48; ++k) shl[k] = (k < n3) ? rw[k - 3] : 0.f;
    }
    if (INFER && a.sh_dir_raw) {
      const float p0[3] = {a.xyz[3 * (size_t)i], a.xyz[3 * (size_t)i + 1], a.xyz[3 * (size_t)i + 2]};
      splat_colour_sh(v, p0, shl, o);
    } else {
      splat_colour_sh(v, act.p, shl, o);
    }
  }
  vis = want;
  if (vis) {
    xy[i] = make_float2(o.px, o.py);
    conic_o[i] = make_float4(o.ca, o.cb, o.cc, act.opac);
    if (!(INFER && a.fwd_only)) rgbd[i] = make_float4(o.rgb[0], o.rgb[1], o.rgb[2], o.depth);
    geo[4 * (size_t)i + 0] = make_float4(o.px, o.py, 0.f, __int_as_float(o.radius));
    geo[4 * (size_t)i + 1] = make_float4(o.ca, o.cb, o.cc, act.opac);
    geo[4 * (size_t)i + 2] = make_float4(o.rgb[0], o.rgb[1], o.rgb[2], o.depth);
    geo[4 * (size_t)i + 3] = split_rgbd(o.rgb[0], o.rgb[1], o.rgb[2], o.depth);
    if (!(INFER && a.fwd_only)) clamped[i] = o.clamped;
  }
  if constexpr (F > 0) {
    constexpr int LPG = F / 4, GPI = 64 / LPG;
    static_assert(LPG == 4 || LPG == 8, "feature width 16 or 32");
    const unsigned long long need = __ballot(active && vis && live);
    const int lane = threadIdx.x & 63;
    float4 r[LPG];
    bool on[LPG];
#pragma unroll
    for (int k = 0; k < LPG; ++k) {
      const int gl = k * GPI + lane / LPG;
      on[k] = (need >> gl) & 1ull;
      r[k] = make_float4(0.f, 0.f, 0.f, 0.f);
      if (on[k]) r[k] = reinterpret_cast<const float4*>(a.features + (size_t)(row0 + gl) * F)[lane % LPG];
    }
#pragma unroll
    for (int k = 0; k < LPG; ++k) {
      float n2 = r[k].x * r[k].x + r[k].y * r[k].y + r[k].z * r[k].z + r[k].w * r[k].w;
      n2 += dpp_f<0xB1>(n2);
      n2 += dpp_f<0x4E>(n2);
      if (LPG == 8) n2 += dpp_f<0x141>(n2);
      const float sc = a.norm_features ? 1.0f / (sqrtf(n2) + 1e-9f) : 1.0f;
      const int gl = k * GPI + lane / LPG;
      if (on[k]) {
        const float4 v = make_float4(r[k].x * sc, r[k].y * sc, r[k].z * sc, r[k].w * sc);
        if (F != 32 || a.write_featn) reinterpret_cast<float4*>(a.featn + (size_t)(row0 + gl) * F)[lane % LPG] = v;
        if constexpr (F == 32) {
          unsigned h01, l01, h23, l23;
          split_pk(v.x, v.y, h01, l01);
          split_pk(v.z, v.w, h23, l23);
          uint32_t* const t = ftab + (size_t)(row0 + gl) * 32 + 2 * (lane % LPG);
          *reinterpret_cast<uint2*>(t) = make_uint2(h01, h23);
          *reinterpret_cast<uint2*>(t + 16) = make_uint2(l01, l23);
        }
      }
    }
  }
}

int launch_preprocess_fwd_raw(const LaunchCtx& c, const TraseRastSettings& s, const TraseRastRawInputs& raw, int32_t* radii,
                              const GeomBuf& g, uint32_t* depth_keys, bool key27, uint32_t key_or, uint32_t key_dead) {
  RawFwdArgs a;
  a.key27 = key27 ? 1 : 0; a.key_or = key_or; a.key_dead = key_dead;
  a.xyz = raw.xyz; a.d_xyz = raw.d_xyz; a.f_dc = raw.features_dc; a.f_rest = raw.features_rest; a.opacity = raw.opacity;
  a.scaling = raw.scaling; a.d_scaling = raw.d_scaling; a.rotation = raw.rotation; a.d_rotation = raw.d_rotation;
  a.features = raw.gaussian_features; a.featn = raw.featn;
  a.write_featn = (c.variant & (TRASE_VARIANT_VALU_BACKWARD | TRASE_VARIANT_VALU_FORWARD)) != 0;
  a.vm = s.viewmatrix; a.pm = s.projmatrix; a.cam = s.campos;
  a.P = raw.P; a.F = raw.F; a.deg = s.sh_degree; a.W = s.image_width; a.H = s.image_height;
  a.norm_features = raw.norm_features; a.tanx = s.tanfovx; a.tany = s.tanfovy; a.mod = s.scale_modifier;
  strip_subtile_rows(s, a.sy_lo, a.sy_hi);
  a.strip = (s.tile_row_begin != 0 || s.tile_row_end != 0) ? 1 : 0;
  a.p_begin = 0; a.p_end = raw.P;
  a.colors = raw.colors_precomp; a.mask = raw.mask; a.se3 = raw.d_xyz_se3; a.sh_dir_raw = raw.sh_dir_undeformed;
  a.fwd_only = 0;
  const bool infer = a.colors || a.mask || a.se3 || a.sh_dir_raw;
  const int blk = a.strip ? 256 : RAW_BLOCK;
  const dim3 grid((raw.P + blk - 1) / blk), block(blk);
  {
    ProfScope ps("preprocess_fwd", c.stream);
#define TRASE_PRF2(FF, BB, II) hipLaunchKernelGGL((preprocess_fwd_raw_kernel<FF, BB, II>), grid, block, 0, c.stream, a, radii, g.xy, g.conic_o, g.rgbd, g.geo, g.ftab, g.tiles, g.clamped, depth_keys, g.hdr)
#define TRASE_PRF(FF) do { if (a.strip) { if (infer) TRASE_PRF2(FF, 256, true); else TRASE_PRF2(FF, 256, false); } \
                           else { if (infer) TRASE_PRF2(FF, RAW_BLOCK, true); else TRASE_PRF2(FF, RAW_BLOCK, false); } } while (0)
    switch (raw.F) {
      case 0: TRASE_PRF(0); break;
      case 16: TRASE_PRF(16); break;
      case 32: TRASE_PRF(32); break;
      default: set_error("preprocess_fwd_raw: feature width %d not compiled in (0,16,32)", raw.F); return TRASE_ERR_UNSUPPORTED;
    }
#undef TRASE_PRF
#undef TRASE_PRF2
  }
  TRASE_POST_LAUNCH("preprocess_fwd", c.stream, c.debug);
  return TRASE_OK;
}

struct RawBwdOut {
  float* d_xyz; float* d_dxyz; float* d_means2D; float* d_f_dc; float* d_f_rest; float* d_opacity;
  float* d_scaling; float* d_dscaling; float* d_rotation; float* d_drotation;
  float* d_colors;
  float* d_se3;
  float* d_feat_zero;
  int F;
};

__device__ __forceinline__ void sh_backward_at(const View& v, const float p_sh[3], const float* sh, unsigned clamped, const float d_rgb[3],
                                               float* d_sh, float d_p_sh[3]) {
  float dr[3];
  for (int ch = 0; ch < 3; ++ch) dr[ch] = ((clamped >> ch) & 1u) ? 0.f : d_rgb[ch];
  float d[3], il, bb[16], gx[16], gy[16], gz[16];
  sh_dir(p_sh, v.cam, d, il);
  sh_basis(v.deg, d, bb);
  sh_basis_grad(v.deg, d, gx, gy, gz);
  float dd[3] = {0.f, 0.f, 0.f};
#pragma unroll
  for (int k = 0; k < 16; ++k) {
    const float s0 = sh[3 * k], s1 = sh[3 * k + 1], s2 = sh[3 * k + 2];
    d_sh[3 * k] = bb[k] * dr[0]; d_sh[3 * k + 1] = bb[k] * dr[1]; d_sh[3 * k + 2] = bb[k] * dr[2];
    const float w = s0 * dr[0] + s1 * dr[1] + s2 * dr[2];
    dd[0] += gx[k] * w; dd[1] += gy[k] * w; dd[2] += gz[k] * w;
  }
  const float dot = d[0] * dd[0] + d[1] * dd[1] + d[2] * dd[2];
  for (int k = 0; k < 3; ++k) d_p_sh[k] = (dd[k] - d[k] * dot) * il;
}

template <bool LIVE, int BLOCK, bool INFER = false>
__global__ __launch_bounds__(BLOCK) void preprocess_bwd_raw_kernel(RawFwdArgs a, const int32_t* __restrict__ radii,
                                                                   const uint32_t* __restrict__ clamped,
                                                                   const uint32_t* __restrict__ tiles,
                                                                   const float* __restrict__ acc, RawBwdOut o,
                                                                   const uint32_t* __restrict__ ids,
                                                                   const uint32_t* __restrict__ n_live_ptr) {
  const int gidx = a.p_begin + blockIdx.x * blockDim.x + threadIdx.x;
  const int p_end = LIVE ? min(a.P, (int)*n_live_ptr) : a.p_end;
  if (LIVE && (gidx & ~63) >= p_end) return;
  const bool active = gidx < p_end;
  const int i = LIVE ? (active ? (int)ids[gidx] : 0) : (active ? gidx : a.P - 1);
  const bool vis = active && radii[i] > 0 && tiles[i] > 0;
  __shared__ __attribute__((aligned(16))) float slabs[BLOCK / 64][REST_SLAB];
  float* const slab = slabs[threadIdx.x >> 6];
  const int row0 = gidx & ~63;
  const bool wave_vis = __ballot(vis) != 0ull;
  const bool precol = INFER && a.colors != nullptr;
  float d_p_raw[3] = {0.f, 0.f, 0.f};
  if (LIVE) {
  } else if (wave_vis && !precol) {
    RestRegs rr;
    rest_rows_load(a.f_rest, row0, a.P, (reinterpret_cast<uintptr_t>(a.f_rest) & 15) == 0, rr);
    rest_rows_to_lds(rr, slab);
  }
  SplatGradOut go;
  float dsh[48];
#pragma unroll
  for (int k = 0; k < 48; ++k) dsh[k] = 0.f;
  SplatGradIn gi;
  gi.d_ndcx = gi.d_ndcy = gi.d_ca = gi.d_cb = gi.d_cc = gi.d_depth = 0.f;
  gi.d_rgb[0] = gi.d_rgb[1] = gi.d_rgb[2] = 0.f;
  float d_op = 0.f;
#pragma unroll
  for (int k = 0; k < 3; ++k) { go.d_p[k] = 0.f; go.d_scale[k] = 0.f; }
#pragma unroll
  for (int k = 0; k < 4; ++k) go.d_quat[k] = 0.f;
  Activated act;
  act.inv_n = 0.f; act.sig = 0.f;
#pragma unroll
  for (int k = 0; k < 3; ++k) act.es[k] = 0.f;
#pragma unroll
  for (int k = 0; k < 4; ++k) act.qn[k] = 0.f;
  if (vis) {
    const float4* r4 = reinterpret_cast<const float4*>(acc + (size_t)i * BWD_ACC);
    const float4 r0 = r4[0], r1 = r4[1], r2 = r4[2];
    gi.d_ndcx = r0.x; gi.d_ndcy = r0.y; gi.d_ca = r0.z; gi.d_cb = r0.w;
    gi.d_cc = r1.x; d_op = r1.y; gi.d_rgb[0] = r1.z; gi.d_rgb[1] = r1.w;
    gi.d_rgb[2] = r2.x; gi.d_depth = r2.y;
    View v;
    raw_view(a, v);
    activate<INFER>(a, i, act);
    float shl[48];
    if (precol) {
    } else if (LIVE) {
      const int n3 = 3 * ncoef(a.deg);
      const float* dc = a.f_dc + 3 * (size_t)i;
      const float* rw = a.f_rest + (size_t)i * REST_W;
      shl[0] = dc[0]; shl[1] = dc[1]; shl[2] = dc[2];
#pragma unroll
      for (int k = 3; k < 48; ++k) shl[k] = (k < n3) ? rw[k - 3] : 0.f;
    } else {
      load_sh_split(a, i, slab, shl);
    }
    const float cv[6] = {0.f, 0.f, 0.f, 0.f, 0.f, 0.f};
    if (precol) {
      splat_backward<false, false>(v, act.p, act.sc, act.q, cv, shl, 0u, gi, go, dsh);
    } else if (INFER && a.sh_dir_raw) {
      const float p0[3] = {a.xyz[3 * (size_t)i], a.xyz[3 * (size_t)i + 1], a.xyz[3 * (size_t)i + 2]};
      splat_backward<false, false>(v, act.p, act.sc, act.q, cv, shl, 0u, gi, go, dsh);
      sh_backward_at(v, p0, shl, clamped[i], gi.d_rgb, dsh, d_p_raw);
    } else {
      splat_backward<false, true>(v, act.p, act.sc, act.q, cv, shl, clamped[i], gi, go, dsh);
    }
  }
  if (active) {
  if (INFER && a.se3) {
    float dx[3] = {0.f, 0.f, 0.f}, dM[16];
#pragma unroll
    for (int k = 0; k < 16; ++k) dM[k] = 0.f;
    if (vis) {
      const float4* M = reinterpret_cast<const float4*>(a.se3) + 4 * (size_t)i;
      const float x = a.xyz[3 * i], y = a.xyz[3 * i + 1], z = a.xyz[3 * i + 2];
      const float4 r0 = M[0], r1 = M[1], r2 = M[2], r3 = M[3];
      const float h3 = r3.x * x + r3.y * y + r3.z * z + r3.w;
      const float inv = 1.0f / h3;
      const float dh[4] = {go.d_p[0] * inv, go.d_p[1] * inv, go.d_p[2] * inv,
                           -(go.d_p[0] * act.p[0] + go.d_p[1] * act.p[1] + go.d_p[2] * act.p[2]) * inv};
      const float ph[4] = {x, y, z, 1.0f};
#pragma unroll
      for (int r = 0; r < 4; ++r)
#pragma unroll
        for (int cc = 0; cc < 4; ++cc) dM[4 * r + cc] = dh[r] * ph[cc];
      dx[0] = dh[0] * r0.x + dh[1] * r1.x + dh[2] * r2.x + dh[3] * r3.x;
      dx[1] = dh[0] * r0.y + dh[1] * r1.y + dh[2] * r2.y + dh[3] * r3.y;
      dx[2] = dh[0] * r0.z + dh[1] * r1.z + dh[2] * r2.z + dh[3] * r3.z;
    }
    if (o.d_xyz) { o.d_xyz[3 * i] = dx[0] + d_p_raw[0]; o.d_xyz[3 * i + 1] = dx[1] + d_p_raw[1]; o.d_xyz[3 * i + 2] = dx[2] + d_p_raw[2]; }
    if (o.d_se3) {
      float4* D = reinterpret_cast<float4*>(o.d_se3) + 4 * (size_t)i;
#pragma unroll
      for (int r = 0; r < 4; ++r) D[r] = make_float4(dM[4 * r], dM[4 * r + 1], dM[4 * r + 2], dM[4 * r + 3]);
    }
  } else {
  if (o.d_xyz) {
    if constexpr (INFER) { o.d_xyz[3 * i] = go.d_p[0] + d_p_raw[0]; o.d_xyz[3 * i + 1] = go.d_p[1] + d_p_raw[1]; o.d_xyz[3 * i + 2] = go.d_p[2] + d_p_raw[2]; }
    else { o.d_xyz[3 * i] = go.d_p[0]; o.d_xyz[3 * i + 1] = go.d_p[1]; o.d_xyz[3 * i + 2] = go.d_p[2]; }
  }
  if (o.d_dxyz) { o.d_dxyz[3 * i] = go.d_p[0]; o.d_dxyz[3 * i + 1] = go.d_p[1]; o.d_dxyz[3 * i + 2] = go.d_p[2]; }
  }
  if (INFER && o.d_colors) { o.d_colors[3 * (size_t)i] = gi.d_rgb[0]; o.d_colors[3 * (size_t)i + 1] = gi.d_rgb[1]; o.d_colors[3 * (size_t)i + 2] = gi.d_rgb[2]; }
  if (o.d_means2D) { o.d_means2D[3 * i] = gi.d_ndcx; o.d_means2D[3 * i + 1] = gi.d_ndcy; o.d_means2D[3 * i + 2] = 0.f; }
  if (o.d_opacity) o.d_opacity[i] = d_op * act.sig * (1.0f - act.sig);
  if (o.d_scaling) {
    o.d_scaling[3 * i] = go.d_scale[0] * act.es[0]; o.d_scaling[3 * i + 1] = go.d_scale[1] * act.es[1];
    o.d_scaling[3 * i + 2] = go.d_scale[2] * act.es[2];
  }
  if (o.d_dscaling) { o.d_dscaling[3 * i] = go.d_scale[0]; o.d_dscaling[3 * i + 1] = go.d_scale[1]; o.d_dscaling[3 * i + 2] = go.d_scale[2]; }
  if (o.d_drotation) reinterpret_cast<float4*>(o.d_drotation)[i] = make_float4(go.d_quat[0], go.d_quat[1], go.d_quat[2], go.d_quat[3]);
  if (o.d_rotation) {
    const float dot = act.qn[0] * go.d_quat[0] + act.qn[1] * go.d_quat[1] + act.qn[2] * go.d_quat[2] + act.qn[3] * go.d_quat[3];
    reinterpret_cast<float4*>(o.d_rotation)[i] =
        make_float4((go.d_quat[0] - act.qn[0] * dot) * act.inv_n, (go.d_quat[1] - act.qn[1] * dot) * act.inv_n,
                    (go.d_quat[2] - act.qn[2] * dot) * act.inv_n, (go.d_quat[3] - act.qn[3] * dot) * act.inv_n);
  }
  if (o.d_f_dc && !precol) { o.d_f_dc[3 * i] = dsh[0]; o.d_f_dc[3 * i + 1] = dsh[1]; o.d_f_dc[3 * i + 2] = dsh[2]; }
  }
  if (o.d_feat_zero) {
    const int lpg = o.F / 4, gpi = 64 / lpg;
    const unsigned long long dead = __ballot(active && !vis);
    const int lane = threadIdx.x & 63;
    for (int k = 0; k < lpg; ++k) {
      const int gl = k * gpi + lane / lpg;
      if ((dead >> gl) & 1ull) reinterpret_cast<float4*>(o.d_feat_zero + (size_t)(row0 + gl) * o.F)[lane % lpg] = make_float4(0.f, 0.f, 0.f, 0.f);
    }
  }
  if (precol) return;
  if (LIVE) {
    if (o.d_f_rest && active) {
      float* rw = o.d_f_rest + (size_t)i * REST_W;
#pragma unroll
      for (int k = 0; k < REST_W; ++k) rw[k] = dsh[3 + k];
    }
    return;
  }
  if (o.d_f_rest) {
    float* row = slab + (threadIdx.x & 63) * REST_W;
#pragma unroll
    for (int k = 0; k < REST_W; ++k) row[k] = dsh[3 + k];
    wave_lds_sync();
    rest_rows_store(o.d_f_rest, row0, a.p_end, (reinterpret_cast<uintptr_t>(o.d_f_rest) & 15) == 0, slab);
  }
}

struct ZeroRowsArgs { float* t[12]; int w[12]; int n; };
__global__ __launch_bounds__(256) void zero_live_rows_kernel(ZeroRowsArgs z, const uint32_t* __restrict__ ids,
                                                             const uint32_t* __restrict__ n_live_ptr, int P) {
  const int n_live = min(P, (int)*n_live_ptr);
  const int t = threadIdx.x & 15;
  for (int k = (blockIdx.x * blockDim.x + threadIdx.x) >> 4; k < n_live; k += (gridDim.x * blockDim.x) >> 4) {
    const size_t id = ids[k];
    for (int j = 0; j < z.n; ++j)
      for (int c = t; c < z.w[j]; c += 16) z.t[j][id * z.w[j] + c] = 0.f;
  }
}

int launch_zero_live_rows(const LaunchCtx& c, const GeomBuf& g, const PreBuf& pre, int P, int F, const TraseRastRawGrads& gr) {
  ZeroRowsArgs z;
  z.n = 0;
  auto add = [&](float* p, int w) { if (p && w > 0) { z.t[z.n] = p; z.w[z.n] = w; ++z.n; } };
  add(gr.dL_dxyz, 3); add(gr.dL_dd_xyz, 3); add(gr.dL_dmeans2D, 3); add(gr.dL_dfeatures_dc, 3); add(gr.dL_dfeatures_rest, 45);
  add(gr.dL_dopacity, 1); add(gr.dL_dscaling, 3); add(gr.dL_dd_scaling, 3); add(gr.dL_drotation, 4); add(gr.dL_dd_rotation, 4);
  add(gr.dL_dgaussian_features, F);
  if (z.n == 0 || P == 0) return TRASE_OK;
  {
    ProfScope ps("zero_live_rows", c.stream);
    const size_t nb = ((size_t)P * 16 + 255) / 256;
    hipLaunchKernelGGL(zero_live_rows_kernel, dim3((int)(nb < 4096 ? nb : 4096)), dim3(256), 0, c.stream, z, pre.live_ids,
                       g.hdr + (HDR_WORDS - 1), P);
  }
  TRASE_POST_LAUNCH("zero_live_rows", c.stream, c.debug);
  return TRASE_OK;
}

int launch_preprocess_bwd_raw(const LaunchCtx& c, const TraseRastSettings& s, const TraseRastRawInputs& raw,
                              const int32_t* radii, const GeomBuf& g, const float* acc, const TraseRastRawGrads& gr,
                              int p_begin, int p_end, int zero_dead_feats, const uint32_t* live_ids) {
  if (p_end < 0) p_end = raw.P;
  if (p_end <= p_begin) return TRASE_OK;
  RawFwdArgs a;
  a.key27 = 0; a.key_or = 0u; a.key_dead = 0u;
  a.write_featn = 0;
  a.p_begin = p_begin; a.p_end = p_end;
  a.xyz = raw.xyz; a.d_xyz = raw.d_xyz; a.f_dc = raw.features_dc; a.f_rest = raw.features_rest; a.opacity = raw.opacity;
  a.scaling = raw.scaling; a.d_scaling = raw.d_scaling; a.rotation = raw.rotation; a.d_rotation = raw.d_rotation;
  a.features = raw.gaussian_features; a.featn = raw.featn;
  a.vm = s.viewmatrix; a.pm = s.projmatrix; a.cam = s.campos;
  a.P = raw.P; a.F = raw.F; a.deg = s.sh_degree; a.W = s.image_width; a.H = s.image_height;
  a.norm_features = raw.norm_features; a.tanx = s.tanfovx; a.tany = s.tanfovy; a.mod = s.scale_modifier;
  strip_subtile_rows(s, a.sy_lo, a.sy_hi);
  RawBwdOut o;
  o.d_xyz = gr.dL_dxyz; o.d_dxyz = gr.dL_dd_xyz; o.d_means2D = gr.dL_dmeans2D; o.d_f_dc = gr.dL_dfeatures_dc;
  o.d_f_rest = gr.dL_dfeatures_rest; o.d_opacity = gr.dL_dopacity; o.d_scaling = gr.dL_dscaling;
  o.d_dscaling = gr.dL_dd_scaling; o.d_rotation = gr.dL_drotation; o.d_drotation = gr.dL_dd_rotation;
  o.d_feat_zero = (zero_dead_feats && (raw.F == 16 || raw.F == 32)) ? gr.dL_dgaussian_features : nullptr; o.F = raw.F;
  o.d_colors = gr.dL_dcolors_precomp; o.d_se3 = gr.dL_dd_xyz_se3;
  a.colors = raw.colors_precomp; a.mask = raw.mask; a.se3 = raw.d_xyz_se3; a.sh_dir_raw = raw.sh_dir_undeformed; a.fwd_only = 0;
  const bool infer = a.colors || a.se3 || a.sh_dir_raw;
  a.strip = 0;
  {
    ProfScope ps("preprocess_bwd", c.stream);
    if (live_ids) {
      if (infer) { set_error("preprocess_bwd_raw: sparse strip gradients are a training path (no override_color / is_6dof / convert_SHs_python)"); return TRASE_ERR_UNSUPPORTED; }
      hipLaunchKernelGGL((preprocess_bwd_raw_kernel<true, 256>), dim3((raw.P + 255) / 256), dim3(256), 0, c.stream, a, radii, g.clamped, g.tiles,
                         acc, o, live_ids, g.hdr + (HDR_WORDS - 1));
    } else if (infer)
      hipLaunchKernelGGL((preprocess_bwd_raw_kernel<false, RAW_BLOCK, true>), dim3((p_end - p_begin + RAW_BLOCK - 1) / RAW_BLOCK), dim3(RAW_BLOCK), 0,
                         c.stream, a, radii, g.clamped, g.tiles, acc, o, nullptr, nullptr);
    else
      hipLaunchKernelGGL((preprocess_bwd_raw_kernel<false, RAW_BLOCK>), dim3((p_end - p_begin + RAW_BLOCK - 1) / RAW_BLOCK), dim3(RAW_BLOCK), 0,
                         c.stream, a, radii, g.clamped, g.tiles, acc, o, nullptr, nullptr);
  }
  TRASE_POST_LAUNCH("preprocess_bwd", c.stream, c.debug);
  return TRASE_OK;
}

}
```

trase_amd/rasterizer.py:

```python
from __future__ import annotations

import ctypes as C
import os
from typing import NamedTuple, Optional

import torch
import torch.nn as nn

from . import _lib


class GaussianRasterizationSettings(NamedTuple):
    image_height: int
    image_width: int
    tanfovx: float
    tanfovy: float
    bg: torch.Tensor
    scale_modifier: float
    viewmatrix: torch.Tensor
    projmatrix: torch.Tensor
    sh_degree: int
    campos: torch.Tensor
    prefiltered: bool
    debug: bool


class _Policy:
    sync = os.environ.get("TRASE_RAST_SYNC", "1") != "0"
    capacity = 0
    variant = int(os.environ.get("TRASE_RAST_VARIANT", "0"), 0)
    last_geom: Optional[torch.Tensor] = None
    last_bin: Optional[torch.Tensor] = None
    last_hw = None
    last_strip = (0, 0)
    guard_reduced = None
    forward_seq = 0
    last_capacity = 0
    pending: list = []
    rollbacks: dict = {}
    max_pending = 8
    tile_rows = (0, 0)
    feat_bg = 0.0


def set_sync(flag: bool, capacity: int = 0):
    _Policy.sync = bool(flag)
    _Policy.capacity = int(capacity)
    _Policy.pending = []
    _Policy.rollbacks = {}


def set_graph(flag="auto"):
    mode = 2 if flag == "auto" else (1 if flag else 0)
    _lib.check(_lib.load().trase_rast_graph_mode(mode), "trase_rast_graph_mode")


def graph_stats() -> dict:
    st = (C.c_int64 * 4)()
    _lib.check(_lib.load().trase_rast_graph_stats(C.byref(st)), "trase_rast_graph_stats")
    return {"hits": int(st[0]), "misses": int(st[1]), "cached": int(st[2]), "enabled": bool(st[3])}


def set_variant(v: int):
    _Policy.variant = int(v)


VARIANT_DEPTH_GRAD, VARIANT_FEATS_BG, VARIANT_DEPTH_NORM = 0x100, 0x10000, 0x20000
VARIANT_FEATURES_ONLY_BWD = 0x400
VARIANT_VALU_BACKWARD, VARIANT_VALU_FORWARD, VARIANT_SLOT_LISTS = 0x40, 0x2000, 0x100000
VARIANT_SPARSE_STRIP_GRADS = 0x200000
VARIANT_FORWARD_ONLY = 0x800000
VARIANT_DEPTH32 = 0x400000


def set_depth_keys(bits: int = 27):
    if bits not in (27, 32):
        raise ValueError("depth keys are 27 or 32 bits")
    _Policy.variant = (_Policy.variant & ~VARIANT_DEPTH32) | (VARIANT_DEPTH32 if bits == 32 else 0)


def set_sparse_strip_grads(flag: bool = True):
    v = _Policy.variant & ~VARIANT_SPARSE_STRIP_GRADS
    _Policy.variant = v | (VARIANT_SPARSE_STRIP_GRADS if flag else 0)


def set_lineage(feats_bg: Optional[float] = None, depth_normalised: bool = False, depth_grad: bool = False):
    v = _Policy.variant & ~(VARIANT_DEPTH_GRAD | VARIANT_FEATS_BG | VARIANT_DEPTH_NORM)
    if feats_bg is not None:
        v |= VARIANT_FEATS_BG
    if depth_normalised:
        v |= VARIANT_DEPTH_NORM
    if depth_grad:
        v |= VARIANT_DEPTH_GRAD
    _Policy.variant = v
    _Policy.feat_bg = 0.0 if feats_bg is None else float(feats_bg)


def set_tile_rows(begin: int = 0, end: int = 0):
    if begin < 0 or end < begin:
        raise ValueError("tile rows must satisfy 0 <= begin <= end")
    _Policy.tile_rows = (int(begin), int(end))


class tile_rows:

    def __init__(self, begin: int, end: int):
        self.rows = (begin, end)

    def __enter__(self):
        self.saved = _Policy.tile_rows
        set_tile_rows(*self.rows)
        return self

    def __exit__(self, *exc):
        _Policy.tile_rows = self.saved


class IterationSkipped(RuntimeError):
    """Raised (by a LATER call: forward, check_overflow) when a sync-free forward turns out to have produced incomplete results
    -- its pair buffer overflowed, or a 27-bit depth key saturated.  The remedy has already been applied (capacity grown / float
    depth keys selected) and the guarded consumers of that iteration skipped it on the device, so a training loop can catch this
    and simply go on::

        try:
            out = render(cam, pc, pipe, bg, d_xyz, d_rot, d_scale)
        except rasterizer.IterationSkipped:
            out = render(cam, pc, pipe, bg, d_xyz, d_rot, d_scale)      # the report concerned an EARLIER iteration

    A RuntimeError subclass: code that catches RuntimeError keeps working."""


def _header_verdict(h, cap: int, what: str):
    r_eff = int(h[2]) & 0xffffffff
    if _Policy.capacity:
        _Policy.capacity = max(_Policy.capacity, int(r_eff * 1.25) + 1024)
    if int(h[16]) or int(h[20]):
        raise RuntimeError(f"trase_amd rasterizer: binning guard tripped in {what} (key flag {int(h[16])}, slot flag {int(h[20])})")
    if int(h[1]) & 2:
        _Policy.variant |= VARIANT_DEPTH32
        raise IterationSkipped(f"trase_amd rasterizer: a Gaussian of {what} lies beyond the range of the 27-bit depth keys (view depth > "
                           f"13 107): that call's depth order was not exact beyond that distance.  This process now sorts on the raw "
                           f"float32 depth bits (rasterizer.set_depth_keys(32)).  Guarded consumers of that iteration "
                           f"(FusedAdam.step, add_densification_stats) skipped it on the device; unguarded ones have used its "
                           f"gradients: re-run the iteration, or call set_depth_keys(32) / set_sync(True) up front for such scenes.")
    if int(h[1]) & 1:
        raise IterationSkipped(f"trase_amd rasterizer: the pair buffer overflowed in {what}: {r_eff} (sub-tile, Gaussian) pairs "
                           f"needed, capacity was {cap}; that call's outputs and gradients were incomplete.  The capacity "
                           f"has been grown to {_Policy.capacity}.  Guarded consumers of that iteration (FusedAdam.step, "
                           f"add_densification_stats) skipped it on the device on every rank (under data parallelism the "
                           f"flag is MAX-reduced over the ranks first): parameters and moments are unchanged.  Consumers "
                           f"that are NOT guarded (torch.optim.Adam, your own statistics) have used the incomplete "
                           f"gradients: re-run the iteration from a checkpoint, or use set_sync(True).")


def _poll_pending(block: bool = False):
    keep = []
    err = None
    for k, (ev, pin, cap) in enumerate(_Policy.pending):
        must = block or (len(_Policy.pending) - k) > _Policy.max_pending
        if must:
            ev.synchronize()
        if must or ev.query():
            undo = _Policy.rollbacks.pop(id(pin), [])
            try:
                _header_verdict(pin.tolist(), cap, "a previous sync-free forward")
            except RuntimeError as e:
                err = err or e
                for fn in undo:
                    fn()
            if len(_PIN_RING) < 16:
                _PIN_RING.append((pin, ev))
        else:
            keep.append((ev, pin, cap))
    _Policy.pending = keep
    if err is not None:
        raise err


def current_guard():
    if _Policy.sync or _Policy.last_geom is None or not _Policy.pending:
        return None
    ev, pin, _cap = _Policy.pending[-1]
    guard = _Policy.last_geom
    import torch.distributed as dist
    if dist.is_available() and dist.is_initialized() and dist.get_world_size() > 1:
        red = _Policy.guard_reduced
        if red is None or red[0] != _Policy.forward_seq:
            buf = guard[:256].view(torch.int32).clone()
            idx = _flag_index(buf.device)
            flags = buf.index_select(0, idx)
            bits = torch.stack([flags[0] & 1, flags[0] & 2])
            flags = torch.cat([flags, bits])
            dist.all_reduce(flags, op=dist.ReduceOp.MAX)
            flags[0] = flags[-2] | flags[-1]
            buf.index_copy_(0, idx, flags[:-2])
            pin.copy_(buf[:32], non_blocking=True)
            if guard.is_cuda:
                ev.record(torch.cuda.current_stream(guard.device))
            _Policy.guard_reduced = red = (_Policy.forward_seq, buf)
        guard = red[1]
    return guard, _Policy.rollbacks.setdefault(id(pin), []).append


_FLAG_WORDS = (1, 2, 16, 20)
_FLAG_INDEX: dict = {}


def _flag_index(device) -> torch.Tensor:
    t = _FLAG_INDEX.get(device)
    if t is None:
        t = _FLAG_INDEX[device] = torch.tensor(_FLAG_WORDS, dtype=torch.int64, device=device)
    return t


def check_overflow():
    _poll_pending(block=True)


def _pick_capacity(lib, ws, stream, rerun_stage1=None) -> int:
    if _Policy.sync or _Policy.capacity <= 0:
        st = (C.c_int64 * 3)()
        _lib.check(lib.trase_rast_status(C.byref(ws), C.byref(st), stream), "trase_rast_status")
        if int(st[1]) & 2 and rerun_stage1 is not None:
            _Policy.variant |= VARIANT_DEPTH32
            rerun_stage1()
            _lib.check(lib.trase_rast_status(C.byref(ws), C.byref(st), stream), "trase_rast_status")
        need = max(int(st[2]), 1)
        if _Policy.sync:
            return need
        _Policy.capacity = int(need * 1.5) + 1024
        return _Policy.capacity
# ... 415 lines not shown
```

Baseline: 923.4.

## Replace 3-pass LSD depth radix sort with range-adaptive MSD bucket sort

During preprocessing, per-wave min/max depth keys are recorded. The sort then uses them to form a single 9-bit histogram and scatter pass over the live key range, followed by a per-bucket local sort in LDS (spilling to global memory for large buckets). This stands in for the three global LSD radix passes of the default 27-bit depth sort and is meant to cut global memory traffic and kernel launches. The costs are an extra per-wave reduction in preprocess, extra complexity, and the risk of load imbalance when depth buckets are skewed. The old path stays available through a variant flag.

```diff
diff --git a/include/trase_rast.h b/include/trase_rast.h
--- a/include/trase_rast.h
+++ b/include/trase_rast.h
@@ -48,6 +48,7 @@
   TRASE_VARIANT_VALU_FORWARD = 0x2000,
   TRASE_VARIANT_SLOT_LISTS = 0x100000,
   TRASE_VARIANT_DEPTH32 = 0x400000,
+  TRASE_VARIANT_DEPTH_LSD = 0x1000000,
   TRASE_VARIANT_FORWARD_ONLY = 0x800000,
   TRASE_VARIANT_SPARSE_STRIP_GRADS = 0x200000,
   TRASE_VARIANT_AB_TIMING = 0x1000,
diff --git a/trase_amd/csrc/api.hip b/trase_amd/csrc/api.hip
--- a/trase_amd/csrc/api.hip
+++ b/trase_amd/csrc/api.hip
@@ -83,6 +83,7 @@
   WsCursor w(ws);
   sort_layout(w, t.sort, p, SORT_KEYS | SORT_VALS);
   t.offsets = w.take<uint32_t>(p);
+  t.krange = t.offsets;
   t.id_end = w.take<uint32_t>(p);
   t.live_ids = w.take<uint32_t>(p);
   t.block_sums = w.take<uint32_t>(3 * partials);
@@ -224,10 +225,12 @@
 
 static int depth_order(const LaunchCtx& c, const TraseRastSettings* s, const GeomBuf& g, const PreBuf& t, int P, const int32_t* radii,
                        int pack_bits) {
-  const DepthSortCfg cfg = depth_sort_cfg(s->variant);
+  const DepthSortCfg cfg = depth_sort_cfg(s->variant, strip_mode(s));
   uint32_t* const flag = cfg.key_bits == 27 ? g.hdr + HDR_OVERFLOW : nullptr;
   int rc, idx = 0;
-  if (strip_mode(s)) {
+  if (cfg.buckets) {
+    rc = depth_bucket_order(c, t.sort, g.hdr + (HDR_WORDS - 1), (uint32_t)P, t.krange, g.hdr);
+  } else if (strip_mode(s)) {
     rc = launch_compact_live(c, g, P, t, t.sort.keys[1 - cfg.start], t.sort.keys[cfg.start], t.sort.vals[cfg.start]);
     if (rc) return rc;
     rc = radix_sort_pairs(c, t.sort, g.hdr + (HDR_WORDS - 1), (uint32_t)P, 0, cfg.key_bits, false, &idx, cfg.digit_bits, cfg.start, DEPTH27_SAT, flag);
@@ -303,8 +306,9 @@
   GeomBuf g; geom_layout(ws->geom, in->P, g);
   PreBuf t; pre_layout(ws->pre, in->P, t);
   if (in->P == 0) return launch_zero_bytes(g.hdr, sizeof(uint32_t) * HDR_WORDS, stream);
-  const DepthSortCfg cfg = depth_sort_cfg(s->variant);
-  rc = launch_preprocess_fwd(c, *s, *in, out->radii, g, t.sort.keys[strip_mode(s) ? 1 - cfg.start : cfg.start], cfg.key_bits == 27);
+  const DepthSortCfg cfg = depth_sort_cfg(s->variant, strip_mode(s));
+  rc = launch_preprocess_fwd(c, *s, *in, out->radii, g, t.sort.keys[strip_mode(s) ? 1 - cfg.start : cfg.start], cfg.key_bits == 27,
+                             cfg.buckets ? t.krange : nullptr);
   if (rc) return rc;
   return depth_order(c, s, g, t, in->P, out->radii, list_pack_bits(s, in->P));
 }
@@ -483,9 +487,9 @@
   GeomBuf g; geom_layout(ws->geom, in.P, g);
   PreBuf t; pre_layout(ws->pre, in.P, t);
   if (in.P == 0) return launch_zero_bytes(g.hdr, sizeof(uint32_t) * HDR_WORDS, stream);
-  const DepthSortCfg cfg = depth_sort_cfg(s->variant);
+  const DepthSortCfg cfg = depth_sort_cfg(s->variant, strip_mode(s));
   rc = launch_preprocess_fwd_raw(c, *s, *raw, out->radii, g, t.sort.keys[strip_mode(s) ? 1 - cfg.start : cfg.start], cfg.key_bits == 27, 0u,
-                                 depth_dead_key(cfg.key_bits == 27));
+                                 depth_dead_key(cfg.key_bits == 27), cfg.buckets ? t.krange : nullptr);
   if (rc) return rc;
   return depth_order(c, s, g, t, in.P, out->radii, list_pack_bits(s, in.P));
 }
diff --git a/trase_amd/csrc/binning.hip b/trase_amd/csrc/binning.hip
--- a/trase_amd/csrc/binning.hip
+++ b/trase_amd/csrc/binning.hip
@@ -13,12 +13,21 @@
 }
 
 template <int DB>
+__device__ __forceinline__ uint32_t bucket_digit(uint32_t key, uint32_t kmin, uint32_t s) {
+  constexpr uint32_t LAST = (1u << DB) - 1u;
+  const uint32_t d = (key - kmin) >> s;
+  return (key == DEPTH27_DEAD || d > LAST) ? LAST : d;
+}
+
+template <int DB, bool BUCKET = false>
 __global__ __launch_bounds__(RS_THREADS) void radix_hist_kernel(const uint32_t* __restrict__ keys,
                                                                 const uint32_t* __restrict__ n_ptr, uint32_t cap,
                                                                 int shift, uint32_t mask, uint32_t* __restrict__ hist,
                                                                 uint32_t* __restrict__ digit_total, int nb_max,
                                                                 uint32_t flag_key = 0u, uint32_t* __restrict__ flag_word = nullptr,
-                                                                uint32_t* __restrict__ zero_from = nullptr, uint32_t zero_words = 0u) {
+                                                                uint32_t* __restrict__ zero_from = nullptr, uint32_t zero_words = 0u,
+                                                                const uint32_t* __restrict__ krange = nullptr,
+                                                                uint32_t* __restrict__ bk_out = nullptr) {
   constexpr int ND = 1 << DB;
   for (uint32_t i = blockIdx.x * RS_THREADS + threadIdx.x; i < zero_words; i += gridDim.x * RS_THREADS) zero_from[i] = 0u;
   const uint32_t n = dev_n(n_ptr, cap);
@@ -27,6 +36,37 @@
   __shared__ uint32_t h[ND];
 #pragma unroll
   for (int d = threadIdx.x; d < ND; d += RS_THREADS) h[d] = 0;
+  uint32_t kmin = 0u, ks = 0u;
+  if constexpr (BUCKET) {
+    __shared__ uint32_t red_mn[RS_WAVES], red_mx[RS_WAVES];
+    const uint2* kr = reinterpret_cast<const uint2*>(krange);
+    const uint32_t nw = (n + 63u) / 64u;
+    uint32_t mn = 0xffffffffu, mx = 0u;
+#pragma unroll 4
+    for (uint32_t w = threadIdx.x; w < nw; w += RS_THREADS) {
+      const uint2 r = kr[w];
+      mn = r.x < mn ? r.x : mn;
+      mx = r.y > mx ? r.y : mx;
+    }
+#pragma unroll
+    for (int o = 32; o > 0; o >>= 1) {
+      const uint32_t a = (uint32_t)__shfl_xor((int)mn, o), b = (uint32_t)__shfl_xor((int)mx, o);
+      mn = a < mn ? a : mn;
+      mx = b > mx ? b : mx;
+    }
+    if ((threadIdx.x & 63) == 0) { red_mn[threadIdx.x >> 6] = mn; red_mx[threadIdx.x >> 6] = mx; }
+    __syncthreads();
+#pragma unroll
+    for (int w = 0; w < RS_WAVES; ++w) { mn = red_mn[w] < mn ? red_mn[w] : mn; mx = red_mx[w] > mx ? red_mx[w] : mx; }
+    if (mn <= mx) {
+      const uint32_t range = mx - mn;
+      const int bits = range ? 32 - __clz((int)range) : 0;
+      ks = bits > DB ? (uint32_t)(bits - DB) : 0u;
+      if ((range >> ks) >= (uint32_t)(ND - 1)) ++ks;
+      kmin = mn;
+    }
+    if (blockIdx.x == 0 && threadIdx.x == 0) { bk_out[0] = kmin; bk_out[1] = ks; }
+  }
   __syncthreads();
   const unsigned lane = threadIdx.x & 63;
   uint32_t kk[RS_ITEMS];
@@ -40,7 +80,7 @@
     const uint32_t idx = base + i * RS_THREADS + threadIdx.x;
     const bool valid = idx < n;
     if (flag_word && valid && kk[i] == flag_key) atomicOr(flag_word, 2u);
-    const uint32_t dg = valid ? ((kk[i] >> shift) & mask) : 0xffffffffu;
+    const uint32_t dg = valid ? (BUCKET ? bucket_digit<DB>(kk[i], kmin, ks) : ((kk[i] >> shift) & mask)) : 0xffffffffu;
     const uint32_t prev = (uint32_t)__shfl_up((int)dg, 1);
     const bool start = valid && (lane == 0 || prev != dg);
     const unsigned long long starts = __ballot(start);
@@ -113,17 +153,20 @@
   if (threadIdx.x == 0) digit_total[d] = carry;
 }
 
-template <bool IOTA, int DB, bool SMALL = false>
+template <bool IOTA, int DB, bool SMALL = false, bool BUCKET = false>
 __global__ __launch_bounds__(RS_THREADS) void radix_scatter_kernel(
     const uint32_t* __restrict__ keys_in, const uint32_t* __restrict__ vals_in, uint32_t* __restrict__ keys_out,
     uint32_t* __restrict__ vals_out, const uint32_t* __restrict__ n_ptr, uint32_t cap, int shift, uint32_t mask,
     const uint32_t* __restrict__ hist, const uint32_t* __restrict__ digit_total, int nb_max,
-    uint32_t* __restrict__ hist_next = nullptr, int shift_next = 0, uint32_t mask_next = 0u) {
+    uint32_t* __restrict__ hist_next = nullptr, int shift_next = 0, uint32_t mask_next = 0u, const uint32_t* __restrict__ bk = nullptr) {
   constexpr int ND = 1 << DB;
   constexpr int DPT = ND / RS_THREADS;
   const uint32_t n = dev_n(n_ptr, cap);
   const uint32_t base = blockIdx.x * RS_TILE;
   if (base >= n) return;
+  uint32_t kmin = 0u, ks = 0u;
+  if constexpr (BUCKET) { kmin = bk[0]; ks = bk[1]; }
+#define TRASE_RS_DIGIT(key) (BUCKET ? bucket_digit<DB>((key), kmin, ks) : (((key) >> shift) & mask))
   __shared__ uint32_t wcount[RS_WAVES][ND];
   const int wave = threadIdx.x >> 6;
   const unsigned lane = threadIdx.x & 63;
@@ -169,7 +212,7 @@
   for (int i = 0; i < RS_ITEMS; ++i) {
     const uint32_t idx = base + wave * RS_SEG + i * WAVE + lane;
     const bool valid = idx < n;
-    const uint32_t dg = (k[i] >> shift) & mask;
+    const uint32_t dg = TRASE_RS_DIGIT(k[i]);
     unsigned long long peers = __ballot(valid);
     const uint32_t dg0 = __builtin_amdgcn_readfirstlane(dg);
     if (!__all(!valid || dg == dg0)) {
@@ -226,7 +269,7 @@
   for (int i = 0; i < RS_ITEMS; ++i) {
     const uint32_t idx = base + wave * RS_SEG + i * WAVE + lane;
     if (idx < n) {
-      const uint32_t dg = (k[i] >> shift) & mask;
+      const uint32_t dg = TRASE_RS_DIGIT(k[i]);
       const uint32_t lp = lstart[dg] + wcount[wave][dg] + rk[i];
       st_k[lp] = k[i];
       st_v[lp] = v[i];
@@ -236,7 +279,7 @@
   const uint32_t nblk = min((uint32_t)RS_TILE, n - base);
   for (uint32_t j = threadIdx.x; j < nblk; j += RS_THREADS) {
     const uint32_t kk = st_k[j];
-    const uint32_t dg = (kk >> shift) & mask;
+    const uint32_t dg = TRASE_RS_DIGIT(kk);
     const uint32_t dst = gbase[dg] + (j - lstart[dg]);
     keys_out[dst] = kk;
     vals_out[dst] = st_v[j];
@@ -255,6 +298,7 @@
       }
     }
   }
+#undef TRASE_RS_DIGIT
 }
 
 __global__ __launch_bounds__(256) void zero_bytes_kernel(uint8_t* __restrict__ p, size_t bytes) {
@@ -376,6 +420,196 @@
   if (digit_bits == 8) return radix_sort_pairs_t<8>(c, t, n_ptr, n_cap, bit_lo, bit_hi, vals_are_iota, start, out_idx, flag_key, flag_word);
   set_error("radix_sort_pairs: digit_bits %d", digit_bits);
   return TRASE_ERR_INVALID;
+}
+
+constexpr int BK_THREADS = 256, BK_WAVES = BK_THREADS / WAVE, BK_ITEMS = BK_CAP / BK_THREADS;
+constexpr int BK_LB = 7, BK_ND = 1 << BK_LB;
+
+template <bool SINGLE>
+__device__ __forceinline__ void bucket_pass(const uint32_t* ksrc, const uint32_t* vsrc, uint32_t* kdst, uint32_t* vdst, uint32_t n,
+                                            uint32_t base, uint32_t shift, uint32_t mask, uint32_t (*wc)[BK_ND], uint32_t* dbase,
+                                            uint32_t* part) {
+  const int t = threadIdx.x, wave = t >> 6;
+  const unsigned lane = t & 63;
+  const unsigned long long lt = lanemask_lt();
+  for (int d = t; d < BK_WAVES * BK_ND; d += BK_THREADS) wc[d / BK_ND][d % BK_ND] = 0u;
+  __syncthreads();
+  const uint32_t per = ((n + BK_THREADS - 1) / BK_THREADS) * WAVE;
+  volatile uint32_t* cnt = wc[wave];
+  uint32_t rk[BK_ITEMS];
+#pragma unroll
+  for (int i = 0; i < BK_ITEMS; ++i) {
+    rk[i] = 0u;
+    if ((uint32_t)i * WAVE < per) {
+      const uint32_t idx = wave * per + i * WAVE + lane;
+      const bool valid = idx < n;
+      const uint32_t dg = valid ? (((ksrc[idx] - base) >> shift) & mask) : 0u;
+      unsigned long long peers = __ballot(valid);
+#pragma unroll
+      for (int bit = 0; bit < BK_LB; ++bit) {
+        const bool set = (dg >> bit) & 1u;
+        const unsigned long long bal = __ballot(set);
+        peers &= set ? bal : ~bal;
+      }
+      const uint32_t in_round = (uint32_t)__popcll(peers & lt);
+      const uint32_t total = (uint32_t)__popcll(peers);
+      uint32_t old = 0;
+      if (valid) {
+        old = cnt[dg];
+        if (in_round == 0) cnt[dg] = old + total;
+      }
+      rk[i] = old + in_round;
+      __builtin_amdgcn_wave_barrier();
+    }
+  }
+  __syncthreads();
+  {
+    uint32_t c[BK_WAVES], tot = 0;
+#pragma unroll
+    for (int w = 0; w < BK_WAVES; ++w) { c[w] = t < BK_ND ? wc[w][t & (BK_ND - 1)] : 0u; tot += c[w]; }
+    uint32_t start;
+    if constexpr (SINGLE) {
+      start = block256_incl_scan(tot, part) - tot;
+    } else {
+      start = t < BK_ND ? dbase[t] : 0u;
+      if (t < BK_ND) dbase[t] = start + tot;
+    }
+    if (t < BK_ND) {
+#pragma unroll
+      for (int w = 0; w < BK_WAVES; ++w) { wc[w][t] = start; start += c[w]; }
+    }
+  }
+  __syncthreads();
+#pragma unroll
+  for (int i = 0; i < BK_ITEMS; ++i) {
+    if ((uint32_t)i * WAVE < per) {
+      const uint32_t idx = wave * per + i * WAVE + lane;
+      if (idx < n) {
+        const uint32_t k = ksrc[idx], v = vsrc[idx];
+        const uint32_t pos = wc[wave][((k - base) >> shift) & mask] + rk[i];
+        kdst[pos] = k;
+        vdst[pos] = v;
+      }
+    }
+  }
+  __syncthreads();
+}
+
+__device__ __forceinline__ void bucket_pass_plan(uint32_t bits, uint32_t& passes, uint32_t& db) {
+  passes = (bits + BK_LB - 1) / BK_LB;
+  db = passes ? (bits + passes - 1) / passes : 0u;
+}
+
+template <int DB>
+__global__ __launch_bounds__(BK_THREADS) void depth_bucket_sort_kernel(uint32_t* keys0, uint32_t* vals0, uint32_t* keys1, uint32_t* vals1,
+                                                                      const uint32_t* __restrict__ digit_total,
+                                                                      const uint32_t* __restrict__ bk) {
+  constexpr int ND = 1 << DB, DPT = ND / BK_THREADS;
+  __shared__ uint32_t off[ND + 1];
+  __shared__ uint32_t part[4], sel[2];
+  __shared__ uint32_t wc[BK_WAVES][BK_ND], dbase[BK_ND];
+  __shared__ uint32_t kb[2][BK_CAP], vb[2][BK_CAP];
+  const int t = threadIdx.x;
+  const uint32_t ks = bk[1];
+  if (ks == 0u) return;
+  const uint32_t kmin = bk[0];
+  uint32_t c[DPT], sum = 0;
+#pragma unroll
+  for (int j = 0; j < DPT; ++j) { c[j] = digit_total[t * DPT + j]; sum += c[j]; }
+  if (t == 0) { sel[0] = (uint32_t)ND; sel[1] = 0u; }
+  uint32_t run = block256_incl_scan(sum, part) - sum;
+#pragma unroll
+  for (int j = 0; j < DPT; ++j) { off[t * DPT + j] = run; run += c[j]; }
+  if (t == BK_THREADS - 1) off[ND] = run;
+  __syncthreads();
+  {
+    const uint32_t g_lo = blockIdx.x * (uint32_t)BK_GROUP, g_hi = g_lo + (uint32_t)BK_GROUP;
+#pragma unroll
+    for (int j = 0; j < DPT; ++j) {
+      const int d = t * DPT + j;
+      const uint32_t o = off[d];
+      if (d < ND - 1 && c[j] > 0u && o >= g_lo && o < g_hi) { atomicMin(&sel[0], (uint32_t)d); atomicMax(&sel[1], (uint32_t)d); }
+    }
+  }
+  __syncthreads();
+  const uint32_t first = sel[0], last = sel[1];
+  if (first == (uint32_t)ND) return;
+  const bool whole = off[last + 1] - off[first] <= (uint32_t)BK_CAP;
+  for (uint32_t d = first; d <= last; d = whole ? last + 1 : d + 1) {
+    const uint32_t d_end = whole ? last : d;
+    const uint32_t lo = off[d], n = off[d_end + 1] - lo;
+    if (n <= 1u) continue;
+    const uint32_t base = kmin + (d << ks);
+    const uint32_t span = ((d_end - d + 1u) << ks) - 1u;
+    uint32_t passes, db;
+    bucket_pass_plan(32u - (uint32_t)__clz((int)span), passes, db);
+    const uint32_t mask = (1u << db) - 1u;
+    if (n <= (uint32_t)BK_CAP) {
+      for (uint32_t j = t; j < n; j += BK_THREADS) { kb[0][j] = keys0[lo + j]; vb[0][j] = vals0[lo + j]; }
+      __syncthreads();
+      uint32_t cur = 0;
+      for (uint32_t p = 0; p < passes; ++p, cur ^= 1u)
+        bucket_pass<true>(kb[cur], vb[cur], kb[cur ^ 1u], vb[cur ^ 1u], n, base, p * db, mask, wc, dbase, part);
+      for (uint32_t j = t; j < n; j += BK_THREADS) vals0[lo + j] = vb[cur][j];
+      __syncthreads();
+    } else {
+      uint32_t* kk[2] = {keys0 + lo, keys1 + lo};
+      uint32_t* vv[2] = {vals0 + lo, vals1 + lo};
+      uint32_t cur = 0;
+      for (uint32_t p = 0; p < passes; ++p, cur ^= 1u) {
+        const uint32_t shift = p * db;
+        if (t < BK_ND) dbase[t] = 0u;
+        __syncthreads();
+        for (uint32_t j = t; j < n; j += BK_THREADS) atomicAdd(&dbase[((kk[cur][j] - base) >> shift) & mask], 1u);
+        __syncthreads();
+        const uint32_t mine = t < BK_ND ? dbase[t] : 0u;
+        const uint32_t ex = block256_incl_scan(mine, part) - mine;
+        if (t < BK_ND) dbase[t] = ex;
+        __syncthreads();
+        for (uint32_t c0 = 0; c0 < n; c0 += (uint32_t)BK_CAP) {
+          const uint32_t nc = n - c0 < (uint32_t)BK_CAP ? n - c0 : (uint32_t)BK_CAP;
+          bucket_pass<false>(kk[cur] + c0, vv[cur] + c0, kk[cur ^ 1u], vv[cur ^ 1u], nc, base, shift, mask, wc, dbase, part);
+        }
+      }
+      if (cur) {
+        for (uint32_t j = t; j < n; j += BK_THREADS) vv[0][j] = vv[1][j];
+      }
+      __syncthreads();
+    }
+  }
+}
+
+int depth_bucket_order(const LaunchCtx& c, const SortBufs& t, const uint32_t* n_ptr, uint32_t n_cap, const uint32_t* krange, uint32_t* hdr) {
+  constexpr int DB = BK_BITS, ND = 1 << DB;
+  static_assert(DB <= DEPTH_MAX_DIGIT_BITS, "the depth sort's histograms are sized for DEPTH_MAX_DIGIT_BITS");
+  const int nb = (int)((n_cap + RS_TILE - 1) / RS_TILE);
+  if (nb > t.nb_max) { set_error("depth_bucket_order: nb %d > nb_max %d", nb, t.nb_max); return TRASE_ERR_WORKSPACE; }
+  uint32_t* const bk = hdr + HDR_KMIN;
+  {
+    ProfScope ps("radix_hist", c.stream);
+    hipLaunchKernelGGL((radix_hist_kernel<DB, true>), dim3(nb), dim3(RS_THREADS), 0, c.stream, t.keys[1], n_ptr, n_cap, 0, 0u, t.hist,
+                       t.digit_total, t.nb_max, DEPTH27_SAT, hdr + HDR_OVERFLOW, (uint32_t*)nullptr, 0u, krange, bk);
+  }
+  TRASE_POST_LAUNCH("radix_hist", c.stream, c.debug);
+  {
+    ProfScope ps("radix_scan", c.stream);
+    hipLaunchKernelGGL(radix_scan_kernel, dim3(ND), dim3(256), 0, c.stream, n_ptr, n_cap, t.hist, t.digit_total, t.nb_max);
+  }
+  TRASE_POST_LAUNCH("radix_scan", c.stream, c.debug);
+  {
+    ProfScope ps("radix_scatter", c.stream);
+    hipLaunchKernelGGL((radix_scatter_kernel<true, DB, false, true>), dim3(nb), dim3(RS_THREADS), 0, c.stream, t.keys[1], t.vals[1], t.keys[0],
+                       t.vals[0], n_ptr, n_cap, 0, 0u, t.hist, t.digit_total, t.nb_max, (uint32_t*)nullptr, 0, 0u, bk);
+  }
+  TRASE_POST_LAUNCH("radix_scatter", c.stream, c.debug);
+  {
+    ProfScope ps("depth_sort", c.stream);
+    const int groups = (int)((n_cap + BK_GROUP - 1) / BK_GROUP);
+    hipLaunchKernelGGL(depth_bucket_sort_kernel<DB>, dim3(groups), dim3(BK_THREADS), 0, c.stream, t.keys[0], t.vals[0], t.keys[1], t.vals[1],
+                       t.digit_total, bk);
+  }
+  TRASE_POST_LAUNCH("depth_sort", c.stream, c.debug);
+  return TRASE_OK;
 }
 
 constexpr int SC_THREADS = 256;
diff --git a/trase_amd/csrc/common.h b/trase_amd/csrc/common.h
--- a/trase_amd/csrc/common.h
+++ b/trase_amd/csrc/common.h
@@ -232,7 +232,7 @@
   return w.bytes();
 }
 
-enum { HDR_R = 0, HDR_OVERFLOW = 1, HDR_R_EFF = 2, HDR_PACK = 3, HDR_WORDS = 64 };
+enum { HDR_R = 0, HDR_OVERFLOW = 1, HDR_R_EFF = 2, HDR_PACK = 3, HDR_KMIN = 24, HDR_KSHIFT = 25, HDR_WORDS = 64 };
 __device__ __forceinline__ uint32_t list_id(uint32_t v, uint32_t jb) { return v >> jb; }
 __device__ __forceinline__ uint32_t list_slot(uint32_t v, uint32_t jb, const uint32_t* id_end, const uint32_t* tiles) {
   const uint32_t id = v >> jb;
@@ -295,6 +295,7 @@
   uint32_t* block_sums;
   uint32_t* block_R;
   uint32_t* block_max;
+  uint32_t* krange;
   uint32_t* live_ids;
 };
 struct PairBuf {
@@ -343,7 +344,7 @@
 int launch_feature_table(const LaunchCtx& c, const float* feats, const uint32_t* tiles, int P, uint32_t* ftab);
 
 int launch_preprocess_fwd(const LaunchCtx& c, const TraseRastSettings& s, const TraseRastInputs& in, int32_t* radii,
-                          const GeomBuf& g, uint32_t* depth_keys, bool key27);
+                          const GeomBuf& g, uint32_t* depth_keys, bool key27, uint32_t* krange = nullptr);
 int launch_preprocess_bwd(const LaunchCtx& c, const TraseRastSettings& s, const TraseRastInputs& in, const int32_t* radii,
                           const GeomBuf& g, const float* acc, const TraseRastGrads& gr);
 
@@ -365,10 +366,13 @@
 int launch_evaluate(const TraseEvalFrame& f, const float* final_T, hipStream_t stream);
 int launch_split_pair_ids(const LaunchCtx& c, const uint32_t* sorted, int P, uint32_t* ids0, uint32_t* ids1);
 int radix_passes(int bit_lo, int bit_hi, int digit_bits = 8);
-struct DepthSortCfg { int key_bits, digit_bits, passes, start; };
-inline DepthSortCfg depth_sort_cfg(int variant) {
-  return (variant & TRASE_VARIANT_DEPTH32) ? DepthSortCfg{32, 8, 4, 0} : DepthSortCfg{27, 9, 3, 1};
-}
+struct DepthSortCfg { int key_bits, digit_bits, passes, start, buckets; };
+inline DepthSortCfg depth_sort_cfg(int variant, bool strip = false) {
+  if (variant & TRASE_VARIANT_DEPTH32) return DepthSortCfg{32, 8, 4, 0, 0};
+  return DepthSortCfg{27, 9, 3, 1, (variant & TRASE_VARIANT_DEPTH_LSD) || strip ? 0 : 1};
+}
+constexpr int BK_BITS = 9, BK_CAP = 4096, BK_GROUP = BK_CAP / 2;
+int depth_bucket_order(const LaunchCtx& c, const SortBufs& t, const uint32_t* n_ptr, uint32_t n_cap, const uint32_t* krange, uint32_t* hdr);
 constexpr int DEPTH_MAX_DIGIT_BITS = 9;
 constexpr uint32_t DEPTH27_BASE = 0x3e4ccccdu, DEPTH27_SAT = 0x07fffffeu, DEPTH27_DEAD = 0x07ffffffu;
 __host__ __device__ inline uint32_t depth_sort_key(float z, bool key27) {
@@ -379,7 +383,18 @@
 }
 inline uint32_t depth_dead_key(bool key27) { return key27 ? DEPTH27_DEAD : 0xffffffffu; }
 int launch_preprocess_fwd_raw(const LaunchCtx& c, const TraseRastSettings& s, const TraseRastRawInputs& raw, int32_t* radii,
-                              const GeomBuf& g, uint32_t* depth_keys, bool key27, uint32_t key_or = 0u, uint32_t key_dead = 0xffffffffu);
+                              const GeomBuf& g, uint32_t* depth_keys, bool key27, uint32_t key_or = 0u, uint32_t key_dead = 0xffffffffu,
+                              uint32_t* krange = nullptr);
+__device__ __forceinline__ void wave_key_range(uint32_t* __restrict__ krange, int wave_id, uint32_t key, bool live) {
+  uint32_t mn = live ? key : 0xffffffffu, mx = live ? key : 0u;
+#pragma unroll
+  for (int o = 32; o > 0; o >>= 1) {
+    const uint32_t a = (uint32_t)__shfl_xor((int)mn, o), b = (uint32_t)__shfl_xor((int)mx, o);
+    mn = a < mn ? a : mn;
+    mx = b > mx ? b : mx;
+  }
+  if ((threadIdx.x & 63) == 0) reinterpret_cast<uint2*>(krange)[wave_id] = make_uint2(mn, mx);
+}
 
 int launch_compact_live(const LaunchCtx& c, const GeomBuf& g, int P, const PreBuf& t, const uint32_t* keys_raw,
                         uint32_t* keys_out, uint32_t* ids_out);
diff --git a/trase_amd/csrc/preprocess.hip b/trase_amd/csrc/preprocess.hip
--- a/trase_amd/csrc/preprocess.hip
+++ b/trase_amd/csrc/preprocess.hip
@@ -16,6 +16,7 @@
   float tanx, tany, mod;
   int sy_lo, sy_hi;
   int key27;
+  uint32_t* krange;
 };
 
 __device__ __forceinline__ void fill_view(const PreArgs& a, View& v) {
@@ -94,6 +95,7 @@
     tiles[i] = live;
     depth_keys[i] = (vis && live) ? depth_sort_key(o.depth, a.key27 != 0) : (a.key27 ? DEPTH27_DEAD : 0xffffffffu);
   }
+  if (a.krange && (gi & ~63) < a.P) wave_key_range(a.krange, gi >> 6, depth_sort_key(o.depth, a.key27 != 0), active && vis && live);
   if (vis) {
     xy[i] = make_float2(o.px, o.py);
     conic_o[i] = make_float4(o.ca, o.cb, o.cc, opac);
@@ -113,13 +115,15 @@
   a.P = in.P; a.M = in.M; a.deg = s.sh_degree; a.W = s.image_width; a.H = s.image_height;
   a.tanx = s.tanfovx; a.tany = s.tanfovy; a.mod = s.scale_modifier;
   strip_subtile_rows(s, a.sy_lo, a.sy_hi);
+  a.key27 = 0; a.krange = nullptr;
 }
 
 int launch_preprocess_fwd(const LaunchCtx& c, const TraseRastSettings& s, const TraseRastInputs& in, int32_t* radii,
-                          const GeomBuf& g, uint32_t* depth_keys, bool key27) {
+                          const GeomBuf& g, uint32_t* depth_keys, bool key27, uint32_t* krange) {
   PreArgs a;
   fill_pre_args(a, s, in);
   a.key27 = key27 ? 1 : 0;
+  a.krange = krange;
   const dim3 grid((in.P + 255) / 256), block(256);
   const bool cov = in.cov3D_precomp != nullptr, sh = in.shs != nullptr;
   {
diff --git a/trase_amd/csrc/preprocess_raw.hip b/trase_amd/csrc/preprocess_raw.hip
--- a/trase_amd/csrc/preprocess_raw.hip
+++ b/trase_amd/csrc/preprocess_raw.hip
@@ -14,6 +14,7 @@
   int strip;
   int p_begin, p_end;
   int key27;
+  uint32_t* krange;
   uint32_t key_or, key_dead;
   const float* colors;
   const uint8_t* mask;
@@ -194,6 +195,7 @@
     tiles[i] = live;
     depth_keys[i] = (vis && live) ? (depth_sort_key(o.depth, a.key27 != 0) | a.key_or) : a.key_dead;
   }
+  if (a.krange) wave_key_range(a.krange, gi >> 6, depth_sort_key(o.depth, a.key27 != 0) | a.key_or, active && vis && live);
   const bool want = vis && (live != 0 || !strip);
   if (!noslab && !precol) {
     rest_rows_to_lds(rr, slab);
@@ -272,9 +274,9 @@
 }
 
 int launch_preprocess_fwd_raw(const LaunchCtx& c, const TraseRastSettings& s, const TraseRastRawInputs& raw, int32_t* radii,
-                              const GeomBuf& g, uint32_t* depth_keys, bool key27, uint32_t key_or, uint32_t key_dead) {
+                              const GeomBuf& g, uint32_t* depth_keys, bool key27, uint32_t key_or, uint32_t key_dead, uint32_t* krange) {
   RawFwdArgs a;
-  a.key27 = key27 ? 1 : 0; a.key_or = key_or; a.key_dead = key_dead;
+  a.key27 = key27 ? 1 : 0; a.key_or = key_or; a.key_dead = key_dead; a.krange = krange;
   a.xyz = raw.xyz; a.d_xyz = raw.d_xyz; a.f_dc = raw.features_dc; a.f_rest = raw.features_rest; a.opacity = raw.opacity;
   a.scaling = raw.scaling; a.d_scaling = raw.d_scaling; a.rotation = raw.rotation; a.d_rotation = raw.d_rotation;
   a.features = raw.gaussian_features; a.featn = raw.featn;
@@ -527,7 +529,7 @@
   if (p_end < 0) p_end = raw.P;
   if (p_end <= p_begin) return TRASE_OK;
   RawFwdArgs a;
-  a.key27 = 0; a.key_or = 0u; a.key_dead = 0u;
+  a.key27 = 0; a.key_or = 0u; a.key_dead = 0u; a.krange = nullptr;
   a.write_featn = 0;
   a.p_begin = p_begin; a.p_end = p_end;
   a.xyz = raw.xyz; a.d_xyz = raw.d_xyz; a.f_dc = raw.features_dc; a.f_rest = raw.features_rest; a.opacity = raw.opacity;
diff --git a/trase_amd/rasterizer.py b/trase_amd/rasterizer.py
--- a/trase_amd/rasterizer.py
+++ b/trase_amd/rasterizer.py
@@ -71,12 +71,17 @@
 VARIANT_SPARSE_STRIP_GRADS = 0x200000
 VARIANT_FORWARD_ONLY = 0x800000
 VARIANT_DEPTH32 = 0x400000
+VARIANT_DEPTH_LSD = 0x1000000
 
 
 def set_depth_keys(bits: int = 27):
     if bits not in (27, 32):
         raise ValueError("depth keys are 27 or 32 bits")
     _Policy.variant = (_Policy.variant & ~VARIANT_DEPTH32) | (VARIANT_DEPTH32 if bits == 32 else 0)
+
+
+def set_depth_buckets(flag: bool = True):
+    _Policy.variant = (_Policy.variant & ~VARIANT_DEPTH_LSD) | (0 if flag else VARIANT_DEPTH_LSD)
 
 
 def set_sparse_strip_grads(flag: bool = True):
```

New measurement: 928.4 (median of 6 runs). About the same (+0.5%).
